# Hi-FT/ERD

Hardware: AMD Instinct MI355X
Metric: images/sec GFL-R50 40+40 incre step @1333x800 (higher is better)
Workload: dtype f32; 1 GPU; gfl_r50_fpn first_40_incre_last_40 ERD (BASELINE configs[1]), 1333x800 padded to 800x1344, fp32, procedural weights; batch_per_gpu=4, global_batch=4, parallelism=dp1

## Files before the change

erd_amd/_lib.py:

```python
from __future__ import annotations

import ctypes as C
import os

_HERE = os.path.dirname(os.path.abspath(__file__))
LIB_PATH = os.environ.get("ERD_HIP_LIB") or os.path.join(_HERE, "lib", "liberd_hip.so")

ERD_MAX_SEG = 5
ERD_MAX_TAPS = 9
ERD_MAX_GROUPS = 8
ERD_SQNORM_PARTS = 1024

c_float_p = C.c_void_p
i64 = C.c_int64
i32 = C.c_int
f32 = C.c_float


class ConvSeg(C.Structure):
    _fields_ = [("inp", C.c_void_p), ("out", C.c_void_p), ("res", C.c_void_p), ("alpha", C.c_void_p),
                ("mask", C.c_void_p), ("N", i32), ("IH", i32), ("IW", i32), ("GH", i32), ("GW", i32), ("OH", i32), ("OW", i32),
                ("in_nstride", i64), ("out_nstride", i64), ("res_nstride", i64),
                ("tap0", i32), ("ntaps", i32), ("oy", i32), ("ox", i32)]


class ConvDesc(C.Structure):
    _fields_ = [("nseg", i32), ("seg", ConvSeg * ERD_MAX_SEG), ("w", C.c_void_p),
                ("Cin", i32), ("Cout", i32), ("wrow", i32), ("ntaps", i32),
                ("dy", i32 * ERD_MAX_TAPS), ("dx", i32 * ERD_MAX_TAPS), ("wk", i32 * ERD_MAX_TAPS),
                ("in_stride", i32), ("out_stride", i32), ("oy", i32), ("ox", i32),
                ("scale", C.c_void_p), ("shift", C.c_void_p), ("relu", i32), ("colsum", C.c_void_p),
                ("sk_ws", C.c_void_p), ("sk_ws_bytes", C.c_size_t), ("w_bf16", C.c_void_p), ("colsum_copies", i32),
                ("in_bf16", i32), ("out_bf16", i32), ("w_x3", C.c_void_p)]


class WgradSeg(C.Structure):
    _fields_ = [("x_off", i64), ("dz_off", i64),
                ("N", i32), ("IH", i32), ("IW", i32), ("GH", i32), ("GW", i32), ("OH", i32), ("OW", i32),
                ("x_nstride", i64), ("dz_nstride", i64)]


class WgradDesc(C.Structure):
    _fields_ = [("x", C.c_void_p), ("dz", C.c_void_p), ("x_elems", i64), ("dz_elems", i64),
                ("nseg", i32), ("seg", WgradSeg * ERD_MAX_SEG),
                ("Cin", i32), ("Cout", i32), ("ntaps", i32),
                ("dy", i32 * ERD_MAX_TAPS), ("dx", i32 * ERD_MAX_TAPS),
                ("in_stride", i32), ("out_stride", i32), ("oy", i32), ("ox", i32),
                ("part", C.c_void_p), ("nsplit", i32), ("bf16_multiplicands", i32),
                ("x_bf16", i32), ("dz_bf16", i32), ("limbs3", i32),
                ("ngroups", i32), ("gx", C.c_void_p * ERD_MAX_GROUPS), ("gdz", C.c_void_p * ERD_MAX_GROUPS)]


class ConvGroupedDesc(C.Structure):
    _fields_ = [("inp", C.c_void_p), ("out", C.c_void_p), ("w", C.c_void_p), ("scale", C.c_void_p), ("shift", C.c_void_p),
                ("res", C.c_void_p), ("mask", C.c_void_p), ("colsum", C.c_void_p), ("colsum_copies", i32),
                ("N", i32), ("IH", i32), ("IW", i32), ("OH", i32), ("OW", i32),
                ("C", i32), ("cg", i32), ("stride", i32), ("relu", i32)]


class WgradReduceGroups(C.Structure):
    _fields_ = [("ngroups", i32), ("w", C.c_void_p * ERD_MAX_GROUPS), ("rowscale", C.c_void_p * ERD_MAX_GROUPS),
                ("dW", C.c_void_p * ERD_MAX_GROUPS), ("rowdot", C.c_void_p * ERD_MAX_GROUPS)]


class BnFoldItem(C.Structure):
    _fields_ = [("gamma", C.c_void_p), ("beta", C.c_void_p), ("mean", C.c_void_p), ("var", C.c_void_p),
                ("scale", C.c_void_p), ("shift", C.c_void_p), ("n", i32), ("eps", f32)]


class WeightPrepItem(C.Structure):
    _fields_ = [("w", C.c_void_p), ("rowscale", C.c_void_p), ("dst", C.c_void_p),
                ("Cout", i32), ("ntaps", i32), ("Cin", i32), ("flip", i32), ("kind", i32), ("block0", i32)]


class ResizeItem(C.Structure):
    _fields_ = [("offset", i64), ("sh", i32), ("sw", i32), ("nh", i32), ("nw", i32), ("flip", i32), ("reserved", i32)]


class Levels(C.Structure):
    _fields_ = [("nseg", i32), ("off", i64 * ERD_MAX_SEG), ("cnt", i64 * ERD_MAX_SEG)]


P = C.c_void_p
_SIGNATURES = {
    "erd_set_cu_reserve": [i32],
    "erd_usable_cus": [],
    "erd_conv_igemm": [C.POINTER(ConvDesc), P],
    "erd_conv_igemm_ws_bytes": [i32],
    "erd_to_bf16": [P, P, i64, P],
    "erd_split3": [P, P, i64, P],
    "erd_conv_thin_enable": [i32],
    "erd_conv_thin_ok": [C.POINTER(ConvDesc)],
    "erd_weight_transpose_x3": [P, P, P, i32, i32, i32, i32, P],
    "erd_wino_weights_elems": [i32, i32],
    "erd_wino_weights": [P, P, i32, i32, i32, P],
    "erd_wino_conv3x3": [P, i32, P, i32, i32, P, P, i32, P, i32, P, P],
    "erd_wino_weights_x3_elems": [i32, i32],
    "erd_wino_weights_x3": [P, P, i32, i32, i32, P],
    "erd_wino_conv3x3_x3": [P, i32, P, i32, i32, P, P, i32, P, i32, P, P],
    "erd_wino_x3_couts_per_item": [P, i32, i32],
    "erd_wino_conv3x3_x3_gn": [P, i32, P, i32, i32, P, P, i32, P, P, C.c_size_t, P],
    "erd_wino_gn_finalize": [P, i32, i32, P, P, f32, P],
    "erd_wino_x3_gn_ws_bytes": [P, i32, i32],
    "erd_conv_wgrad": [C.POINTER(WgradDesc), P],
    "erd_wgrad_row3_slices": [C.POINTER(WgradDesc)],
    "erd_conv_grouped_fwd": [C.POINTER(ConvGroupedDesc), P],
    "erd_conv_grouped_dgrad": [C.POINTER(ConvGroupedDesc), P],
    "erd_conv_grouped_wgrad": [P, P, P, i32, i32, i32, i32, i32, i32, i32, P],
    "erd_conv_grouped_wgrad_splits": [i32, i32, i32, i32, i32, i32],
    "erd_deform_cols": [P, P, P, i32, i32, i32, i32, i32, P],
    "erd_deform_cols_bwd": [P, P, P, P, P, i32, i32, i32, i32, i32, P],
    "erd_wgrad_reduce": [P, i32, i32, i32, P, P, P, i32, P, P],
    "erd_wgrad_reduce_rows": [P, i32, i32, i32, i32, P, i32, P],
    "erd_wgrad_reduce_grouped": [P, i32, i32, i32, C.POINTER(WgradReduceGroups), i32, P],
    "erd_conv_wgrad_wino": [C.POINTER(WgradDesc), P],
    "erd_conv_wgrad_wino_ok": [C.POINTER(WgradDesc)],
    "erd_conv_wgrad_wino_tile": [C.POINTER(WgradDesc)],
    "erd_wgrad_wino_reduce": [P, i32, i32, i32, P, i32, P],
    "erd_weight_transpose": [P, P, P, i32, i32, i32, i32, P],
    "erd_weight_transpose_bf16": [P, P, P, i32, i32, i32, i32, P],
    "erd_stem_conv7x7_bn_relu": [P, P, P, P, P, i32, i32, i32, P],
    "erd_maxpool3x3s2": [P, P, i32, i32, i32, i32, i32, P],
    "erd_bn_fold": [P, P, P, P, f32, P, P, i64, P],
    "erd_bn_fold_batch": [P, i32, i32, P],
    "erd_weight_prep_blocks": [i32, i32, i32, i32],
    "erd_weight_prep_batch": [P, i32, i32, P],
    "erd_relu_bwd_colsum": [P, P, P, i64, i32, i64, i64, P, i32, i32, P],
    "erd_bn_dgamma": [P, P, i32, P, P, f32, P, P, i32, i32, P],
    "erd_gn_relu_fwd": [P, P, P, P, P, P, i32, i64, i32, i32, C.POINTER(Levels), f32, i32, P],
    "erd_gn_relu_apply": [P, P, P, P, P, i32, i64, i32, i32, C.POINTER(Levels), i32, P],
    "erd_gn_relu_bwd": [P, P, P, P, P, P, P, P, P, i32, i64, i32, i32, C.POINTER(Levels), i32, P],
    "erd_upsample2x_add": [P, P, i32, i32, i32, i32, i32, i32, i64, i64, i32, P],
    "erd_upsample2x_add_bwd": [P, P, i32, i32, i32, i32, i32, i32, i64, i64, i32, P],
    "erd_colsum": [P, i64, i32, P, i32, i32, P],
    "erd_pad_channels": [P, P, i64, i32, i32, P],
    "erd_level_scale": [P, P, P, i32, i64, i32, C.POINTER(Levels), P],
    "erd_level_scale_bwd": [P, P, P, P, P, i32, i64, i32, C.POINTER(Levels), P],
    "erd_sgd_momentum": [P, P, P, i64, f32, f32, f32, f32, i32, P],
    "erd_sgd_groups_table": [P, P, P, i32, P, P],
    "erd_sgd_momentum_groups": [P, P, P, i64, i64, P, i32, i32, i64, i64, f32, f32, f32, P, i32, P],
    "erd_adam_groups": [P, P, P, P, i64, i64, P, i32, i32, i64, i64, f32, f32, C.c_double, C.c_double, f32, f32, f32, f32, P, i32, P],
    "erd_grad_sqnorm": [P, i64, P, P],
    "erd_clip_coef": [P, i32, f32, f32, P, P],
    "erd_grad_accumulate": [P, P, i64, i32, P],
    "erd_ers_select": [P, P, i32, i64, i32, i32, P, P, P, P, P, P, P, P],
    "erd_grid_anchors": [P, C.POINTER(i32), C.POINTER(i32), C.POINTER(i32), i32, i32, P],
    "erd_atss_assign": [P, P, C.POINTER(i64), i32, i64, P, P, P, i32, i32, i32, i32, P, P, P, P, P, P],
    "erd_gfl_losses_fwd": [P, P, P, P, P, P, C.POINTER(i64), C.POINTER(i32), i32, i32, i64, i32, i32, P, P, P, P],
    "erd_gfl_losses_bwd": [P, P, P, P, P, P, C.POINTER(i64), C.POINTER(i32), i32, i32, i64, i32, i32, P, P, P, P,
                           P, P],
    "erd_l2_distill": [P, P, P, P, i32, i64, i32, i32, i32, P, P],
    "erd_l2_distill_bwd": [P, P, P, P, P, i32, i64, i32, i32, i32, P, P],
    "erd_distill_nms": [P, P, P, P, P, i32, i64, i32, f32, P, P, P, C.c_size_t, P],
    "erd_kd_kl": [P, P, P, P, i32, i64, i32, i32, f32, P, P],
    "erd_kd_kl_bwd": [P, P, P, P, P, i32, i64, i32, i32, f32, P, P],
    "erd_loss_avg": [P, i32, P, i32, P, P],
    "erd_loss_finalize": [P, P, P, P, P, i32, i32, i32, f32, f32, f32, f32, f32, P, P, P, P],
    "erd_preprocess_image": [P, i32, i32, i32, P, i32, i32, P, P, i32, f32, P],
    "erd_resize_normalize": [P, i32, i32, P, P, P, P, i32, i32, P, i32, i32, P, P, i32, i32, f32, P],
    "erd_resize_normalize_batch": [P, i64, P, i32, P, i32, i32, P, P, i32, f32, P],
    "erd_predict_ws_bytes": [i32, i32, i32],
    "erd_predict_topk": [P, P, P, i32, i64, i32, P, P, P, f32, i32, P, P, P, P, P, C.c_size_t, P],
    "erd_predict_nms": [P, P, P, P, i32, i32, P, f32, f32, i32, P, P, P, P, C.c_size_t, P],
    "erd_tta_merge_ws_bytes": [i32, i32, i32],
    "erd_tta_merge": [P, P, P, i32, i32, i32, P, P, f32, i32, P, P, P, P, C.c_size_t, P],
    "erd_coco_dets_append": [P, P, P, P, i32, i32, P, P, P, P, P],
    "erd_coco_eval_ws_bytes": [i64, i32, i32, i64],
    "erd_coco_eval": [P, P, P, P, i64, P, P, P, P, i32, i32, i64, P, P, P, P, P, P, P, P, C.c_size_t, P],
    "erd_qfl_rows": [P, P, P, i64, i32, P, P],
    "erd_qfl_bwd": [P, P, P, P, i64, i32, P, P],
    "erd_dfl": [P, P, P, i64, i32, P, P, P],
    "erd_kd_kl_rows": [P, P, P, i64, i32, f32, P, P, P],
    "erd_giou": [P, P, P, i64, f32, P, P, P],
    "erd_bbox_overlaps": [P, P, i64, i64, i32, i32, f32, P, P],
    "erd_integral": [P, P, i64, i32, P, P, P],
    "erd_distance2bbox": [P, P, P, i64, f32, f32, P, P, P],
    "erd_bbox2distance": [P, P, i64, f32, f32, P, P],
    "erd_weighted_sum": [P, P, i64, C.c_double, P, P],
    "erd_loss_coef": [P, P, i64, f32, P, P],
    "erd_rows_mul": [P, P, i64, f32, P, P],
    "erd_atss_result": [P, P, i64, P, P, P, P],
}

EXPORTS = ["erd_abi_version", "erd_probe_build", "erd_last_error", "erd_csrc_sha"] + sorted(_SIGNATURES)

_lib = None


class ErdHipError(RuntimeError):
    pass


def load():
    global _lib
    if _lib is not None:
        return _lib
    if not os.path.isfile(LIB_PATH):
        raise ErdHipError(
            f"{LIB_PATH} is missing: build it with `python -c 'import __graft_entry__ as g; g.build()'` "
            "(or `make -C erd_amd/csrc`).  erd_amd has no CPU fallback.")
    lib = C.CDLL(LIB_PATH)
    lib.erd_abi_version.restype = C.c_int
    lib.erd_last_error.restype = C.c_char_p
    lib.erd_csrc_sha.restype = C.c_char_p
    for name, args in _SIGNATURES.items():
        fn = getattr(lib, name)
        fn.argtypes = args
        fn.restype = C.c_size_t if name.endswith(("_ws_bytes", "_elems")) else C.c_int
    if lib.erd_abi_version() != 6:
        raise ErdHipError("liberd_hip.so ABI version mismatch")
    lib.erd_probe_build.restype = C.c_int
    if lib.erd_probe_build() and not os.environ.get("ERD_HIP_LIB"):
        raise ErdHipError(f"{LIB_PATH} is a PROBE build (a kernel was compiled with a timing / accuracy / trace macro of "
                          "csrc/erd_probes.h): rebuild with `make -C erd_amd/csrc`, or select it explicitly with ERD_HIP_LIB")
    _lib = lib
    return lib


def call(name: str, *args) -> None:
    lib = load()
    rc = getattr(lib, name)(*args)
    if rc != 0:
        raise ErdHipError(f"{name} failed (rc={rc}): {lib.erd_last_error().decode(errors='replace')}")
```

erd_amd/csrc/wgrad_wino.hip:

```cpp
#include <stdlib.h>
#include "erd_common.h"

namespace {

typedef float f32x16 __attribute__((ext_vector_type(16)));
typedef __bf16 bf16x8 __attribute__((ext_vector_type(8)));
typedef unsigned int u4v __attribute__((ext_vector_type(4)));
typedef unsigned int u2v __attribute__((ext_vector_type(2)));

constexpr int WT = 512;
constexpr int KT = 16;
constexpr int BC = 128;
constexpr int ROWB = 2 * KT;
constexpr int PLANE = BC * ROWB;
constexpr int LIMB = 2 * PLANE;
constexpr int POS = 3 * LIMB;
constexpr int OPER_BYTES = 4 * POS;
constexpr int TAB_U = 8, NSLOT = 4;
constexpr size_t LDS_BYTES = OPER_BYTES + NSLOT * KT * TAB_U * sizeof(unsigned);
constexpr unsigned INV = 0x80000000u;

__device__ __forceinline__ float2 buf_load8(__amdgpu_buffer_rsrc_t r, unsigned byte_off) {
    const u2v v = __builtin_amdgcn_raw_buffer_load_b64(r, byte_off, 0, 0);
    return make_float2(__uint_as_float(v.x), __uint_as_float(v.y));
}
__device__ __forceinline__ float2 buf_load8(__amdgpu_buffer_rsrc_t r, unsigned byte_off, unsigned uniform_off) {
    const u2v v = __builtin_amdgcn_raw_buffer_load_b64(r, byte_off, uniform_off, 0);
    return make_float2(__uint_as_float(v.x), __uint_as_float(v.y));
}
__device__ __forceinline__ float comp(const float2& v, int c) { return c == 0 ? v.x : v.y; }

struct WinoMap { int xb, zb, IH, IW, OH, OW; };

__device__ __forceinline__ int tiles_w(const erd_wgrad_seg& g) { return (g.GW + 1) >> 1; }
__device__ __forceinline__ int tiles_h(const erd_wgrad_seg& g) { return (g.GH + 1) >> 1; }

struct Sel {
    int xa, xb, za;
    float sx, sz, cz;
    bool z_two;
    __device__ __forceinline__ explicit Sel(int r)
        : xa(r), xb(r < 2 ? 2 : 1), za(r == 3 ? 1 : 0), sx(r == 1 ? 1.f : -1.f), sz(r == 2 ? -1.f : 1.f), cz(r == 1 || r == 2 ? 0.5f : 1.f),
          z_two(r == 1 || r == 2) {}
};

struct TileTable {
    const erd_wgrad_desc& p;
    const Sel& rs;
    const Sel& cs;
    unsigned* tab;
    int lane, ntiles;
    int sl, sn = 0, sa = 0, sb = 0;
    __device__ __forceinline__ TileTable(const erd_wgrad_desc& p_, const Sel& rs_, const Sel& cs_, unsigned* tab_, int lane_, int ntiles_)
        : p(p_), rs(rs_), cs(cs_), tab(tab_), lane(lane_), ntiles(ntiles_), sl(p_.nseg) {}

    __device__ __forceinline__ void tile_entry(const WinoMap& m, int ty, int tx, unsigned (&ent)[5]) const {
        const int ra = 2 * ty - 1 + rs.xa, rb = 2 * ty - 1 + rs.xb, c0 = 2 * tx - 1;
        if ((unsigned)ra < (unsigned)m.IH) ent[0] = (unsigned)(m.xb + (ra * m.IW + c0) * p.Cin) * 4u;
        if ((unsigned)rb < (unsigned)m.IH) ent[1] = (unsigned)(m.xb + (rb * m.IW + c0) * p.Cin) * 4u;
        const int qa = 2 * ty + rs.za, qb = 2 * ty + 1;
        if (qa < m.OH) ent[2] = (unsigned)(m.zb + (qa * m.OW + 2 * tx) * p.Cout) * 4u;
        if (rs.z_two && qb < m.OH) ent[3] = (unsigned)(m.zb + (qb * m.OW + 2 * tx) * p.Cout) * 4u;
        unsigned mask = 0;
#pragma unroll
        for (int b = 0; b < 4; ++b) mask |= (unsigned)(c0 + b) < (unsigned)m.IW ? 1u << b : 0u;
        mask |= (2 * tx < m.OW ? 16u : 0u) | (2 * tx + 1 < m.OW ? 32u : 0u);
        ent[4] = mask;
    }
    __device__ __forceinline__ void tile_entry_pos(const WinoMap& m, int ty, int tx, unsigned (&ent)[8]) const {
        const int ra = 2 * ty - 1 + rs.xa, rb = 2 * ty - 1 + rs.xb, ca = 2 * tx - 1 + cs.xa, cb = 2 * tx - 1 + cs.xb;
        const bool ra_in = (unsigned)ra < (unsigned)m.IH, rb_in = (unsigned)rb < (unsigned)m.IH;
        const bool ca_in = (unsigned)ca < (unsigned)m.IW, cb_in = (unsigned)cb < (unsigned)m.IW;
        if (ra_in && ca_in) ent[0] = (unsigned)(m.xb + (ra * m.IW + ca) * p.Cin) * 4u;
        if (ra_in && cb_in) ent[1] = (unsigned)(m.xb + (ra * m.IW + cb) * p.Cin) * 4u;
        if (rb_in && ca_in) ent[2] = (unsigned)(m.xb + (rb * m.IW + ca) * p.Cin) * 4u;
        if (rb_in && cb_in) ent[3] = (unsigned)(m.xb + (rb * m.IW + cb) * p.Cin) * 4u;
        const int qa = 2 * ty + rs.za, qb = 2 * ty + 1, ka = 2 * tx + cs.za, kb = 2 * tx + 1;
        const bool qb_in = rs.z_two && qb < m.OH, kb_in = cs.z_two && kb < m.OW;
        if (qa < m.OH && ka < m.OW) ent[4] = (unsigned)(m.zb + (qa * m.OW + ka) * p.Cout) * 4u;
        if (qa < m.OH && kb_in) ent[5] = (unsigned)(m.zb + (qa * m.OW + kb) * p.Cout) * 4u;
        if (qb_in && ka < m.OW) ent[6] = (unsigned)(m.zb + (qb * m.OW + ka) * p.Cout) * 4u;
        if (qb_in && kb_in) ent[7] = (unsigned)(m.zb + (qb * m.OW + kb) * p.Cout) * 4u;
    }
    static __device__ __forceinline__ WinoMap map_of(const erd_wgrad_seg& g, int n) {
        return WinoMap{(int)(g.x_off + n * g.x_nstride), (int)(g.dz_off + n * g.dz_nstride), g.IH, g.IW, g.OH, g.OW};
    }
    __device__ __forceinline__ void locate(int u, int& l, int& n, int& a, int& b) const {
        l = 0;
#pragma unroll 1
        for (; l < p.nseg - 1; ++l) {
            const int cnt = p.seg[l].N * tiles_h(p.seg[l]) * tiles_w(p.seg[l]);
            if (u < cnt) break;
            u -= cnt;
        }
        const int TW = tiles_w(p.seg[l]), THW = tiles_h(p.seg[l]) * TW;
        n = u / THW;
        const int rem = u - n * THW;
        a = rem / TW;
        b = rem - a * TW;
    }
    __device__ __forceinline__ void start(int g) {
        if (g * KT < ntiles) locate(g * KT, sl, sn, sa, sb);
    }
    template <bool POS, int SPAN = KT>
    __device__ __forceinline__ void build(int g, int slot) {
        sl = __builtin_amdgcn_readfirstlane(sl);
        sn = __builtin_amdgcn_readfirstlane(sn);
        sa = __builtin_amdgcn_readfirstlane(sa);
        sb = __builtin_amdgcn_readfirstlane(sb);
        if (lane < SPAN) {
            unsigned ent[8] = {INV, INV, INV, INV, POS ? INV : 0u, INV, INV, INV};
            auto entry = [&](const WinoMap& m, int a, int b) {
                if constexpr (POS) tile_entry_pos(m, a, b, ent);
                else tile_entry(m, a, b, reinterpret_cast<unsigned (&)[5]>(ent));
            };
            if (sl < p.nseg) {
                const erd_wgrad_seg& sg = p.seg[sl];
                const int TW = tiles_w(sg);
                int a = sa, b = sb + lane;
                while (b >= TW) { b -= TW; ++a; }
                if (a < tiles_h(sg)) entry(map_of(sg, sn), a, b);
                else if (g * KT + lane < ntiles) {
                    int l, n;
                    locate(g * KT + lane, l, n, a, b);
                    entry(map_of(p.seg[l], n), a, b);
                }
            }
            unsigned* e = tab + (slot * KT + lane) * TAB_U;
            *reinterpret_cast<u4v*>(e) = u4v{ent[0], ent[1], ent[2], ent[3]};
            if constexpr (POS) *reinterpret_cast<u4v*>(e + 4) = u4v{ent[4], ent[5], ent[6], ent[7]};
            else e[4] = ent[4];
        }
        sb += SPAN;
        while (sl < p.nseg && sb >= tiles_w(p.seg[sl])) {
            sb -= tiles_w(p.seg[sl]);
            const bool img = sa + 1 == tiles_h(p.seg[sl]);
            sa = img ? 0 : sa + 1;
            const bool seg = img && sn + 1 == p.seg[sl].N;
            sn = seg ? 0 : sn + (img ? 1 : 0);
            sl += seg ? 1 : 0;
        }
    }
};

__global__ __launch_bounds__(WT) void conv_wgrad_wino_kernel(const erd_wgrad_desc p, const int ntiles, const int nsteps) {
    extern __shared__ __attribute__((aligned(16))) char smem[];
    unsigned* tab = reinterpret_cast<unsigned*>(smem + OPER_BYTES);

    const int tid = threadIdx.x, wave = tid >> 6, lane = tid & 63;
    const int wave_u = __builtin_amdgcn_readfirstlane(wave);

    const int nci = p.Cin / BC, nco = p.Cout / BC, ncomb = 4 * nci * nco;
    const int wg = erd::xcd_contiguous(blockIdx.x, gridDim.x);
    const int split = wg / ncomb, comb = wg - split * ncomb;
    const int r = comb & 3, ct = comb >> 2;
    const int ci0 = (ct % nci) * BC, co0 = (ct / nci) * BC;
    const int per = (nsteps + p.nsplit - 1) / p.nsplit;
    const int g_begin = split * per, g_end = min(nsteps, g_begin + per);

    const Sel rs(r);
    const float sx = rs.sx, sz = rs.sz, cz = rs.cz;
    const bool z_two = rs.z_two;
    TileTable tt{p, rs, rs, tab, lane, ntiles};

    const int cg = (wave & 3) * 16 + (lane & 15), tp = (wave >> 2) * 4 + (lane >> 4);
    const __amdgpu_buffer_rsrc_t rs_x = __builtin_amdgcn_make_buffer_rsrc(const_cast<float*>(p.x), 0, (int)(p.x_elems * 4), 0x00020000);
    const __amdgpu_buffer_rsrc_t rs_z = __builtin_amdgcn_make_buffer_rsrc(const_cast<float*>(p.dz), 0, (int)(p.dz_elems * 4), 0x00020000);
    const unsigned chan_x = (unsigned)(ci0 + 2 * cg) * 4u, chan_z = (unsigned)(co0 + 2 * cg) * 4u;
    const unsigned step_x = (unsigned)p.Cin * 4u, step_z = (unsigned)p.Cout * 4u;
    float2 rx[16], rz[8];
#pragma unroll
    for (int i = 0; i < 8; ++i) rz[i] = make_float2(0.f, 0.f);
    auto load_global = [&](int slot) {
#pragma unroll
        for (int q = 0; q < 2; ++q) {
            const unsigned* e = tab + (slot * KT + 2 * tp + q) * TAB_U;
            const u4v o = *reinterpret_cast<const u4v*>(e);
            const unsigned mask = e[4];
#pragma unroll
            for (int w = 0; w < 2; ++w)
#pragma unroll
                for (int b = 0; b < 4; ++b) {
                    const bool ok = o[w] != INV && ((mask >> b) & 1u);
                    rx[q * 8 + w * 4 + b] = buf_load8(rs_x, ok ? o[w] + (unsigned)b * step_x + chan_x : INV);
                }
#pragma unroll
            for (int w = 0; w < 2; ++w) {
                if (w == 1 && !z_two) continue;
#pragma unroll
                for (int b = 0; b < 2; ++b) {
                    const bool ok = o[2 + w] != INV && ((mask >> (4 + b)) & 1u);
                    rz[q * 4 + w * 2 + b] = buf_load8(rs_z, ok ? o[2 + w] + (unsigned)b * step_z + chan_z : INV);
                }
            }
        }
    };
    char* const st_base = smem + cg * ROWB + ((((tp >> 2) ^ (cg >> 3)) & 1) << 4) + ((tp & 3) << 2);
    auto store_limbs = [&](char* dst, const float (&v)[2][4]) {
#pragma unroll
        for (int j = 0; j < 4; ++j) {
            unsigned hi, mid, lo;
            erd::limbs3_pair(v[0][j], v[1][j], hi, mid, lo);
            *reinterpret_cast<unsigned*>(dst + j * POS) = hi;
            *reinterpret_cast<unsigned*>(dst + j * POS + LIMB) = mid;
            *reinterpret_cast<unsigned*>(dst + j * POS + 2 * LIMB) = lo;
        }
    };
    auto store_lds = [&]() {
#pragma unroll
        for (int c = 0; c < 2; ++c) {
            float v[2][4];
#pragma unroll
            for (int q = 0; q < 2; ++q) {
                float t[4];
#pragma unroll
                for (int b = 0; b < 4; ++b) t[b] = __builtin_fmaf(sx, comp(rx[q * 8 + 4 + b], c), comp(rx[q * 8 + b], c));
                v[q][0] = t[0] - t[2];
                v[q][1] = t[1] + t[2];
                v[q][2] = t[2] - t[1];
                v[q][3] = t[3] - t[1];
            }
            store_limbs(st_base + PLANE + c * (64 * ROWB), v);
#pragma unroll
            for (int q = 0; q < 2; ++q) {
                float t[2];
#pragma unroll
                for (int b = 0; b < 2; ++b) t[b] = cz * __builtin_fmaf(sz, comp(rz[q * 4 + 2 + b], c), comp(rz[q * 4 + b], c));
                v[q][0] = t[0];
                v[q][1] = 0.5f * (t[0] + t[1]);
                v[q][2] = 0.5f * (t[0] - t[1]);
                v[q][3] = t[1];
            }
            store_limbs(st_base + c * (64 * ROWB), v);
        }
    };

    const int pj = wave & 3, half = wave >> 2;
    const int li = lane & 31, h = lane >> 5;
    f32x16 acc[2][4];
#pragma unroll
    for (int i = 0; i < 2; ++i)
#pragma unroll
        for (int j = 0; j < 4; ++j)
#pragma unroll
            for (int e = 0; e < 16; ++e) acc[i][j][e] = 0.f;

    if (g_begin < g_end) {
        if (wave_u == 0) {
            tt.start(g_begin);
            tt.build<false>(g_begin, 0);
            tt.build<false>(g_begin + 1, 1);
        }
        __syncthreads();
        load_global(0);
        store_lds();
        __syncthreads();
        const char* const fr = smem + pj * POS + li * ROWB + (((h ^ (li >> 3)) & 1) << 4);
        for (int g = g_begin; g < g_end; ++g) {
            const int k = g - g_begin;
            const bool more = g + 1 < g_end;
#ifndef ERD_WW_NOLOAD
            if (more) load_global((k + 1) & (NSLOT - 1));
#endif
#ifndef ERD_WW_NOTABLE
            if (wave_u == 0 && g + 2 < g_end) tt.build<false>(g + 2, (k + 2) & (NSLOT - 1));
#endif
#ifndef ERD_WW_NOMFMA
            u4v fa[2][3];
#pragma unroll
            for (int pl = 0; pl < 3; ++pl)
#pragma unroll
                for (int i = 0; i < 2; ++i) fa[i][pl] = *reinterpret_cast<const u4v*>(fr + pl * LIMB + (half * 2 + i) * (32 * ROWB));
#pragma unroll
            for (int jh = 0; jh < 2; ++jh) {
                u4v fb[2][3];
#pragma unroll
                for (int pl = 0; pl < 3; ++pl)
#pragma unroll
                    for (int j = 0; j < 2; ++j) fb[j][pl] = *reinterpret_cast<const u4v*>(fr + pl * LIMB + PLANE + (jh * 2 + j) * (32 * ROWB));
#define ERD_W3(APL, BPL)                                                                                                                     \
    _Pragma("unroll") for (int j = 0; j < 2; ++j) _Pragma("unroll") for (int i = 0; i < 2; ++i) acc[i][jh * 2 + j] =                         \
        __builtin_amdgcn_mfma_f32_32x32x16_bf16(__builtin_bit_cast(bf16x8, fa[i][APL]), __builtin_bit_cast(bf16x8, fb[j][BPL]), acc[i][jh * 2 + j], 0, 0, 0);
                ERD_W3(0, 2) ERD_W3(0, 1) ERD_W3(1, 1) ERD_W3(2, 0) ERD_W3(1, 0) ERD_W3(0, 0)
#undef ERD_W3
            }
#endif
            __syncthreads();
#ifndef ERD_WW_NOSPLIT
            if (more) store_lds();
#endif
            __syncthreads();
        }
    }

    float* __restrict__ part = p.part + ((int64_t)(split * 16 + 4 * r + pj) * p.Cout) * p.Cin;
#pragma unroll
    for (int i = 0; i < 2; ++i)
#pragma unroll
        for (int e = 0; e < 16; ++e) {
            const int co = co0 + 2 * (32 * i + (e & 3) + 8 * (e >> 2) + 4 * h) + half;
            float* row = part + (int64_t)co * p.Cin + ci0 + 2 * li;
            *reinterpret_cast<float2*>(row) = make_float2(acc[i][0][e], acc[i][2][e]);
            *reinterpret_cast<float2*>(row + 64) = make_float2(acc[i][1][e], acc[i][3][e]);
        }
}

constexpr int BP = 256;
constexpr int PPLANE = BP * ROWB;
constexpr int PLIMB = 2 * PPLANE;
constexpr int POPER_BYTES = 3 * PLIMB;
constexpr unsigned PBUF_XOR = 65536;
constexpr int PSPAN = 4 * KT, PNSLOT = 8;
constexpr size_t PTAB_BYTES = PNSLOT * KT * TAB_U * sizeof(unsigned);
constexpr size_t PLDS_BYTES = PBUF_XOR + POPER_BYTES;
static_assert(POPER_BYTES + PTAB_BYTES <= PBUF_XOR, "the table lies between the buffers");

__global__ __launch_bounds__(WT) void wgrad_wino_pos_kernel(const erd_wgrad_desc p, const int ntiles, const int nsteps) {
    extern __shared__ __attribute__((aligned(16))) char smem[];
    unsigned* tab = reinterpret_cast<unsigned*>(smem + POPER_BYTES);

    const int tid = threadIdx.x, wave = tid >> 6, lane = tid & 63;
    const int wave_u = __builtin_amdgcn_readfirstlane(wave);

    const int nci = p.Cin / BP, nco = p.Cout / BP, ncomb = 16 * nci * nco;
    const int wg = erd::xcd_contiguous(blockIdx.x, gridDim.x);
    const int split = wg / ncomb, comb = wg - split * ncomb;
    const int xi = comb & 15, ct = comb >> 4;
    const int ci0 = (ct % nci) * BP, co0 = (ct / nci) * BP;
    const int per = (nsteps + p.nsplit - 1) / p.nsplit;
    const int g_begin = split * per, g_end = min(nsteps, g_begin + per);

    const Sel rs(xi >> 2), cs(xi & 3);
    const float sx = rs.sx, sz = rs.sz, cz = rs.cz;
    const bool z_two = rs.z_two, zc_two = cs.z_two;
    const float sxc = cs.sx, szc = cs.sz;
    TileTable tt{p, rs, cs, tab, lane, ntiles};

    const int cg = wave * 16 + (lane & 15), tq = lane >> 4;
    const __amdgpu_buffer_rsrc_t rs_x = __builtin_amdgcn_make_buffer_rsrc(const_cast<float*>(p.x), 0, (int)(p.x_elems * 4), 0x00020000);
    const __amdgpu_buffer_rsrc_t rs_z = __builtin_amdgcn_make_buffer_rsrc(const_cast<float*>(p.dz), 0, (int)(p.dz_elems * 4), 0x00020000);
    const unsigned chan = (unsigned)cg * 8u, tile_x = (unsigned)ci0 * 4u, tile_z = (unsigned)co0 * 4u;
    float2 rx[16], rz[16];
#pragma unroll
    for (int i = 0; i < 16; ++i) rz[i] = make_float2(0.f, 0.f);
    auto load_global = [&](int slot) {
        u4v ox[4], oz[4];
#pragma unroll
        for (int q = 0; q < 4; ++q) {
            const unsigned* e = tab + (slot * KT + 4 * tq + q) * TAB_U;
            ox[q] = *reinterpret_cast<const u4v*>(e);
            oz[q] = *reinterpret_cast<const u4v*>(e + 4);
        }
#pragma unroll
        for (int q = 0; q < 4; ++q)
#pragma unroll
            for (int i = 0; i < 4; ++i) rx[q * 4 + i] = buf_load8(rs_x, ox[q][i] + chan, tile_x);
#pragma unroll
        for (int q = 0; q < 4; ++q) rz[q * 4] = buf_load8(rs_z, oz[q][0] + chan, tile_z);
        if (zc_two) {
#pragma unroll
            for (int q = 0; q < 4; ++q) rz[q * 4 + 1] = buf_load8(rs_z, oz[q][1] + chan, tile_z);
        }
        if (z_two) {
#pragma unroll
            for (int q = 0; q < 4; ++q) rz[q * 4 + 2] = buf_load8(rs_z, oz[q][2] + chan, tile_z);
            if (zc_two) {
#pragma unroll
                for (int q = 0; q < 4; ++q) rz[q * 4 + 3] = buf_load8(rs_z, oz[q][3] + chan, tile_z);
            }
        }
    };
    unsigned st_off = cg * ROWB + ((((tq >> 1) ^ (cg >> 3)) & 1) << 4) + ((tq & 1) << 3);
    auto store_limbs = [&](char* dst, const float (&v)[4]) {
        unsigned hi[2], mid[2], lo[2];
        erd::limbs3_pair(v[0], v[1], hi[0], mid[0], lo[0]);
        erd::limbs3_pair(v[2], v[3], hi[1], mid[1], lo[1]);
        *reinterpret_cast<u2v*>(dst) = u2v{hi[0], hi[1]};
        *reinterpret_cast<u2v*>(dst + PLIMB) = u2v{mid[0], mid[1]};
        *reinterpret_cast<u2v*>(dst + 2 * PLIMB) = u2v{lo[0], lo[1]};
    };
    auto store_lds = [&]() {
        char* const st = smem + st_off;
#pragma unroll
        for (int c = 0; c < 2; ++c) {
            float v[4];
#pragma unroll
            for (int q = 0; q < 4; ++q) {
                const float ta = __builtin_fmaf(sx, comp(rx[q * 4 + 2], c), comp(rx[q * 4], c));
                const float tb = __builtin_fmaf(sx, comp(rx[q * 4 + 3], c), comp(rx[q * 4 + 1], c));
                v[q] = __builtin_fmaf(sxc, tb, ta);
            }
            store_limbs(st + PPLANE + c * (128 * ROWB), v);
#pragma unroll
            for (int q = 0; q < 4; ++q) {
                const float ta = cz * __builtin_fmaf(sz, comp(rz[q * 4 + 2], c), comp(rz[q * 4], c));
                const float tb = cz * __builtin_fmaf(sz, comp(rz[q * 4 + 3], c), comp(rz[q * 4 + 1], c));
                v[q] = zc_two ? 0.5f * __builtin_fmaf(szc, tb, ta) : ta;
            }
            store_limbs(st + c * (128 * ROWB), v);
        }
    };

    const int zq = wave >> 1, hx = wave & 1;
    const int li = lane & 31, h = lane >> 5;
    f32x16 acc[2][4];
#pragma unroll
    for (int i = 0; i < 2; ++i)
#pragma unroll
        for (int j = 0; j < 4; ++j)
#pragma unroll
            for (int e = 0; e < 16; ++e) acc[i][j][e] = 0.f;

    if (g_begin < g_end) {
        if (wave_u == 0) {
            tt.start(g_begin);
            tt.build<true, PSPAN>(g_begin, 0);
            tt.build<true, PSPAN>(g_begin + 4, 4);
        }
        __syncthreads();
        load_global(0);
        store_lds();
        __syncthreads();
        st_off ^= PBUF_XOR;
        unsigned fr_off = li * ROWB + (((h ^ (li >> 3)) & 1) << 4);
        for (int g = g_begin; g < g_end; ++g) {
            const int k = g - g_begin;
            const bool more = g + 1 < g_end;
            const char* const fr = smem + fr_off;
#ifndef ERD_WW_NOLOAD
            if (more) load_global((k + 1) & (PNSLOT - 1));
#endif
#ifndef ERD_WW_NOTABLE
            if (wave_u == 0 && (k & 3) == 3 && g + 5 < g_end) tt.build<true, PSPAN>(g + 5, (k + 5) & (PNSLOT - 1));
#endif
#ifndef ERD_WW_NOMFMA
            u4v fa[2][3];
#pragma unroll
            for (int pl = 0; pl < 3; ++pl)
#pragma unroll
                for (int i = 0; i < 2; ++i) fa[i][pl] = *reinterpret_cast<const u4v*>(fr + pl * PLIMB + (zq * 2 + i) * (32 * ROWB));
#pragma unroll
            for (int j = 0; j < 4; ++j) {
                u4v fb[3];
#pragma unroll
                for (int pl = 0; pl < 3; ++pl)
                    fb[pl] = *reinterpret_cast<const u4v*>(fr + pl * PLIMB + PPLANE + (2 * hx + (j & 1) + 4 * (j >> 1)) * (32 * ROWB));
#define ERD_W3(APL, BPL)                                                                                                                     \
    _Pragma("unroll") for (int i = 0; i < 2; ++i) acc[i][j] =                                                                                \
        __builtin_amdgcn_mfma_f32_32x32x16_bf16(__builtin_bit_cast(bf16x8, fa[i][APL]), __builtin_bit_cast(bf16x8, fb[BPL]), acc[i][j], 0, 0, 0);
                ERD_W3(0, 2) ERD_W3(0, 1) ERD_W3(1, 1) ERD_W3(2, 0) ERD_W3(1, 0) ERD_W3(0, 0)
#undef ERD_W3
            }
#endif
#ifndef ERD_WW_NOSPLIT
            if (more) store_lds();
#endif
            __syncthreads();
            fr_off ^= PBUF_XOR;
            st_off ^= PBUF_XOR;
        }
    }

    float* __restrict__ part = p.part + ((int64_t)(split * 16 + xi) * p.Cout) * p.Cin;
#pragma unroll
    for (int i = 0; i < 2; ++i)
#pragma unroll
        for (int e = 0; e < 16; ++e) {
            const int co = co0 + 2 * (32 * (2 * (zq & 1) + i) + (e & 3) + 8 * (e >> 2) + 4 * h) + (zq >> 1);
            float* row = part + (int64_t)co * p.Cin + ci0 + 2 * (64 * hx + li);
            *reinterpret_cast<float2*>(row) = make_float2(acc[i][0][e], acc[i][2][e]);
            *reinterpret_cast<float2*>(row + 64) = make_float2(acc[i][1][e], acc[i][3][e]);
        }
}

__global__ __launch_bounds__(256) void wgrad_wino_reduce_kernel(const float* __restrict__ part, int nsplit, int Cout, int Cin,
                                                                 float* __restrict__ dW, int accumulate) {
    __shared__ float4 du[16][16];
    const int co = blockIdx.x, xi = threadIdx.x >> 4, c4 = threadIdx.x & 15;
    const int ci = blockIdx.y * 64 + c4 * 4;
    const int64_t slab = (int64_t)16 * Cout * Cin;
    float4 s = make_float4(0.f, 0.f, 0.f, 0.f);
    if (ci < Cin) {
        const float* src = part + ((int64_t)xi * Cout + co) * Cin + ci;
        for (int k = 0; k < nsplit; ++k) {
            const float4 v = *reinterpret_cast<const float4*>(src + k * slab);
            s.x += v.x; s.y += v.y; s.z += v.z; s.w += v.w;
        }
    }
    du[xi][c4] = s;
    __syncthreads();
    if (threadIdx.x >= 9 * 16 || ci >= Cin) return;
    const int a = xi / 3, b = xi - 3 * a;
    auto col = [&](int i) {
        const float4 u1 = du[4 * i + 1][c4], u2 = du[4 * i + 2][c4];
        if (b == 1) return make_float4(u1.x - u2.x, u1.y - u2.y, u1.z - u2.z, u1.w - u2.w);
        const float4 u0 = du[4 * i + (b == 0 ? 0 : 3)][c4];
        return make_float4((u1.x + u2.x) + u0.x, (u1.y + u2.y) + u0.y, (u1.z + u2.z) + u0.z, (u1.w + u2.w) + u0.w);
    };
    const float4 e1 = col(1), e2 = col(2);
    float4 o;
    if (a == 1) o = make_float4(e1.x - e2.x, e1.y - e2.y, e1.z - e2.z, e1.w - e2.w);
    else {
        const float4 e0 = col(a == 0 ? 0 : 3);
        o = make_float4((e1.x + e2.x) + e0.x, (e1.y + e2.y) + e0.y, (e1.z + e2.z) + e0.z, (e1.w + e2.w) + e0.w);
    }
    float* dst = dW + ((int64_t)co * 9 + xi) * Cin + ci;
    if (accumulate) {
        const float4 old = *reinterpret_cast<const float4*>(dst);
        o.x += old.x; o.y += old.y; o.z += old.z; o.w += old.w;
    }
    *reinterpret_cast<float4*>(dst) = o;
}

int64_t wino_tiles(const erd_wgrad_desc* d) {
    int64_t n = 0;
    for (int l = 0; l < d->nseg; ++l) n += (int64_t)d->seg[l].N * ((d->seg[l].GH + 1) / 2) * ((d->seg[l].GW + 1) / 2);
    return n;
}

int wino_tile(const erd_wgrad_desc* d) {
    const bool can = d->Cin % BP == 0 && d->Cout % BP == 0;
    const char* const e = getenv("ERD_WGRAD_WINO_TILE");
    const int force = e ? atoi(e) : 0;
    if (force == BC || !can) return BC;
    return BP;
}

}

extern "C" int erd_conv_wgrad_wino_tile(const erd_wgrad_desc* d) { return erd_conv_wgrad_wino_ok(d) ? wino_tile(d) : 0; }

extern "C" int erd_conv_wgrad_wino_ok(const erd_wgrad_desc* d) {
    if (!d || d->bf16_multiplicands || d->x_bf16 || d->dz_bf16 || d->ngroups != 1) return 0;
    if (d->nseg < 1 || d->nseg > ERD_MAX_SEG || d->Cin < BC || d->Cout < BC || d->Cin % BC || d->Cout % BC) return 0;
    if (d->x_elems <= 0 || d->dz_elems <= 0 || d->x_elems >= (1ll << 29) || d->dz_elems >= (1ll << 29)) return 0;
    for (int l = 0; l < d->nseg; ++l)
        if (d->seg[l].N < 1 || d->seg[l].GH < 1 || d->seg[l].GW < 1) return 0;
    return erd_wgrad_row3_slices(d) > 0 && wino_tiles(d) < (1ll << 30);
}

extern "C" int erd_conv_wgrad_wino(const erd_wgrad_desc* d, erd_stream_t stream) {
    ERD_REQUIRE(d != nullptr && d->part && d->x && d->dz, "wgrad_wino: null pointer");
    ERD_REQUIRE(!d->bf16_multiplicands && !d->x_bf16 && !d->dz_bf16, "wgrad_wino: fp32 maps and the three-limb form only");
    ERD_REQUIRE(d->ngroups == 1, "wgrad_wino: ngroups=%d", d->ngroups);
    ERD_REQUIRE(d->Cin >= BC && d->Cout >= BC && d->Cin % BC == 0 && d->Cout % BC == 0, "wgrad_wino: Cin=%d Cout=%d must be multiples of %d", d->Cin,
                d->Cout, BC);
    ERD_REQUIRE(d->in_stride == 1 && d->out_stride == 1, "wgrad_wino: stride 1 only");
    ERD_REQUIRE(erd_conv_wgrad_wino_ok(d), "wgrad_wino: not a 3x3 / stride 1 / pad 1 layer over 1 .. %d non-empty maps below 2 GiB", ERD_MAX_SEG);
    const int64_t grid = (int64_t)4 * (d->Cin / BC) * (d->Cout / BC) * d->nsplit;
    ERD_REQUIRE(d->nsplit >= 1 && grid < (1 << 20), "wgrad_wino: nsplit=%d", d->nsplit);
    const int ntiles = (int)wino_tiles(d), nsteps = (ntiles + KT - 1) / KT;
    static bool attr_done = false;
    if (!attr_done) {
        (void)hipFuncSetAttribute(reinterpret_cast<const void*>(conv_wgrad_wino_kernel), hipFuncAttributeMaxDynamicSharedMemorySize, (int)LDS_BYTES);
        (void)hipFuncSetAttribute(reinterpret_cast<const void*>(wgrad_wino_pos_kernel), hipFuncAttributeMaxDynamicSharedMemorySize, (int)PLDS_BYTES);
        attr_done = true;
    }
    if (wino_tile(d) == BP) hipLaunchKernelGGL(wgrad_wino_pos_kernel, dim3((unsigned)grid), dim3(WT), PLDS_BYTES, (hipStream_t)stream, *d, ntiles, nsteps);
    else hipLaunchKernelGGL(conv_wgrad_wino_kernel, dim3((unsigned)grid), dim3(WT), LDS_BYTES, (hipStream_t)stream, *d, ntiles, nsteps);
    return erd::check_launch("conv_wgrad_wino");
}

extern "C" int erd_wgrad_wino_reduce(const float* part, int nsplit, int Cout, int Cin, float* dW, int accumulate, erd_stream_t stream) {
    ERD_REQUIRE(part && dW && nsplit >= 1 && Cout >= 1 && Cin >= 4 && Cin % 4 == 0, "wgrad_wino_reduce: bad args");
    hipLaunchKernelGGL(wgrad_wino_reduce_kernel, dim3(Cout, (Cin + 63) / 64), dim3(256), 0, (hipStream_t)stream, part, nsplit, Cout, Cin, dW,
                       accumulate & 1);
    return erd::check_launch("wgrad_wino_reduce");
}
```

erd_amd/functional.py:

```python
from __future__ import annotations

from typing import List, Optional, Sequence, Tuple

import torch
from torch.autograd import Function

from . import kernels as K

Tensor = torch.Tensor


def ohwi(w: Tensor) -> Tensor:
    v = w.detach().permute(0, 2, 3, 1)
    if not v.is_contiguous():
        return v.contiguous()
    v._erd_owner = w
    return v


def _to_oihw(dw_ohwi: Tensor) -> Tensor:
    return dw_ohwi.permute(0, 3, 1, 2)


_AUX = {}
import contextlib as _contextlib
import os as _os
WGRAD_ON_AUX_STREAM = _os.environ.get('ERD_WGRAD_AUX', '0') != '0'
TOWERS_ON_TWO_STREAMS = _os.environ.get('ERD_TOWER_AUX', '1') != '0'


_TOWER = {}

CAPTURE_ORIGIN = None


def _may_fork(cur) -> bool:
    return CAPTURE_ORIGIN is None or cur.cuda_stream == CAPTURE_ORIGIN


WGRAD_TRAIL = _os.environ.get('ERD_WGRAD_TRAIL', '1') != '0'
WGRAD_GROUPED = _os.environ.get('ERD_WGRAD_GROUPED', '1') != '0'
WGRAD_WINO = _os.environ.get('ERD_WGRAD_WINO', '1') != '0'
WGRAD_GROUP_CAP = 8
RES_LAYER_NODE = _os.environ.get('ERD_RES_LAYER', '1') != '0'
HEAD_TRAIL = _os.environ.get('ERD_HEAD_TRAIL', '0') != '0'
_TRAIL = {}
_TRAIL_ACTIVE = set()


def trail_stream(device) -> "torch.cuda.Stream":
    key = str(torch.device(device))
    if key not in _TRAIL:
        _TRAIL[key] = torch.cuda.Stream(device=device)
    return _TRAIL[key]


def trail_join(device=None) -> None:
    for key in list(_TRAIL_ACTIVE):
        if device is None or key == str(torch.device(device)):
            torch.cuda.current_stream(torch.device(key)).wait_stream(_TRAIL[key])
            _TRAIL_ACTIVE.discard(key)


class _Trail:

    def __init__(self, device, *tensors):
        self.cur = torch.cuda.current_stream(device)
        self.aux = trail_stream(device)
        self.tensors = [t for t in tensors if t is not None]
        self.key = str(torch.device(device))
        self.inline = not _may_fork(self.cur)

    def __enter__(self):
        if self.inline:
            return self
        self.aux.wait_stream(self.cur)
        for t in self.tensors:
            t.record_stream(self.aux)
        _TRAIL_ACTIVE.add(self.key)
        self.ctx = torch.cuda.stream(self.aux)
        self.ctx.__enter__()
        return self

    def __exit__(self, *a):
        if not self.inline:
            self.ctx.__exit__(*a)
        return False


def aux_stream(device) -> "torch.cuda.Stream":
    cur = torch.cuda.current_stream(device)
    if not TOWERS_ON_TWO_STREAMS or not _may_fork(cur):
        return cur
    key = (str(device), cur.cuda_stream)
    if key not in _TOWER:
        _TOWER[key] = torch.cuda.Stream(device=device)
    return _TOWER[key]


class _Fork:
    def __init__(self, device):
        self.cur = torch.cuda.current_stream(device)
        key = (str(device), self.cur.cuda_stream)
        if key not in _AUX:
            _AUX[key] = torch.cuda.Stream(device=device)
        self.aux = _AUX[key] if WGRAD_ON_AUX_STREAM and _may_fork(self.cur) else None

    def __enter__(self):
        if self.aux is not None:
            self.aux.wait_stream(self.cur)
            self.ctx = torch.cuda.stream(self.aux)
            self.ctx.__enter__()
        return self

    def __exit__(self, *a):
        if self.aux is not None:
            self.ctx.__exit__(*a)
        return False

    def join(self):
        if self.aux is not None:
            self.cur.wait_stream(self.aux)


def _sink(p: Optional[Tensor]) -> Optional[Tensor]:
    if p is not None and getattr(p, "_erd_sink", False) and p.grad is not None:
        return p.grad
    return None


def _sunk(p: Tensor) -> None:
    n = getattr(p, "_erd_sink_notify", None)
    if n is not None:
        n(p)


def _emit_wgrad(w: Tensor, part: Tensor, S: int, wk: Tensor, scale: Optional[Tensor], rowdot: Optional[Tensor]):
    sink = _sink(w)
    if sink is not None:
        K.wgrad_reduce(part, S, wk, scale, ohwi(sink), True, rowdot, rowdot_zeroed=True)
        _sunk(w)
        return None
    dWk = torch.empty_like(wk)
    K.wgrad_reduce(part, S, wk, scale, dWk, False, rowdot, rowdot_zeroed=True)
    return _to_oihw(dWk)


def _emit_wgrad_wino(w: Tensor, part: Tensor, S: int, wk: Tensor):
    sink = _sink(w)
    if sink is not None:
        K.wgrad_wino_reduce(part, S, ohwi(sink), True)
        _sunk(w)
        return None
    dWk = torch.empty_like(wk)
    K.wgrad_wino_reduce(part, S, dWk, False)
    return _to_oihw(dWk)


class _WgradGroups:

    def __init__(self, device, eps: float):
        self.dev, self.eps, self.keys = device, eps, {}
        self.launches = []

    @staticmethod
    def takes(xin: Tensor, dz: Tensor, cardinality: int = 1) -> bool:
        if cardinality > 1:
            return False
        return WGRAD_GROUPED and CAPTURE_ORIGIN is None and K.COMPUTE == "f32x3" and K.WGRAD_X3 and K.WGRAD_X3_GENERIC and xin.dtype == torch.float32 \
            and dz.dtype == torch.float32 and _os.environ.get("ERD_WGRAD_ROW3", "1") != "0"

    def add(self, single, xin, dz, k, s, pad, scale, dbeta, prm, need3) -> None:
        key = (k, s, pad, xin.shape, xin.stride(), dz.shape, dz.stride())
        q = self.keys.setdefault(key, [])
        q.append((single, xin, dz, k, s, pad, scale, dbeta, prm, need3))
        if len(q) == WGRAD_GROUP_CAP:
            self._launch(self.keys.pop(key))

    def flush(self) -> None:
        for key in list(self.keys):
            self._launch(self.keys.pop(key))

    def _launch(self, q) -> None:
        self.launches.append(len(q))
        if len(q) == 1:
            q[0][0]()
            return
        _, _, _, k, s, pad = q[0][:6]
        with (_Trail(self.dev, *[t for m in q for t in (m[1], m[2], m[6], m[7])]) if WGRAD_TRAIL else _contextlib.nullcontext()):
            part, S = K.conv_wgrad_partials_grouped([[m[1]] for m in q], [[m[2]] for m in q], k, s, pad)
            wks = [ohwi(m[8][0]) for m in q]
            rowdots = [K.zeros_f32(m[6].numel(), m[6].device) if m[9][1] else None for m in q]
            K.wgrad_reduce_grouped(part, S, wks, [m[6] for m in q], [ohwi(_sink(m[8][0])) for m in q], True, rowdots, rowdot_zeroed=True)
            for m, rowdot in zip(q, rowdots):
                (w, g, b, mean, var), (_, need_g, need_b), dbeta = m[8], m[9], m[7]
                _sunk(w)
                if need_g:
                    rep = dbeta.dim() == 2
                    bs_fold = (_sink(b) if need_b else None) if rep else None
                    fold = None if not rep else (bs_fold if bs_fold is not None else torch.empty_like(dbeta[0]))
                    K.bn_dgamma(rowdot, dbeta, mean, var, self.eps, out=_sink(g), dbeta_out=fold)
                    _sunk(g)
                    if rep:
                        dbeta = fold
                elif dbeta.dim() == 2:
                    dbeta = dbeta.sum(0)
                if need_b:
                    bs = _sink(b)
                    if dbeta.data_ptr() != bs.data_ptr():
                        bs.add_(dbeta)
                    _sunk(b)


def _bn_fold_cached(gamma, beta, mean, var, eps):
    if gamma.requires_grad or beta.requires_grad:
        pre = getattr(gamma, "_erd_prefold", None)
        if pre is not None and pre[0] == (gamma.data_ptr(), beta.data_ptr(), mean.data_ptr(), var.data_ptr(), gamma._version,
                                         beta._version, mean._version, var._version, eps) and pre[1][0]:
            return pre[2], pre[3]
        return K.bn_fold(gamma.detach(), beta.detach(), mean, var, eps)
    ver = (gamma.data_ptr(), beta.data_ptr(), mean.data_ptr(), var.data_ptr(),
           gamma._version, beta._version, mean._version, var._version, eps)
    hit = getattr(gamma, "_erd_fold", None)
    if hit is None or hit[0] != ver:
        hit = (ver, K.bn_fold(gamma.detach(), beta.detach(), mean, var, eps))
        gamma._erd_fold = hit
    return hit[1]


class BnPrefold:

    def __init__(self, model):
        from ._lib import BnFoldItem
        bns = [m for m in model.modules() if hasattr(m, "running_var") and hasattr(m, "weight") and m.weight is not None
               and (m.weight.requires_grad or m.bias.requires_grad)]
        self.bns = bns
        self.valid = [False]
        if not bns:
            return
        dev = bns[0].weight.device
        total = sum(m.weight.numel() for m in bns)
        self.buf = torch.empty(2 * total, dtype=torch.float32, device=dev)
        items = (BnFoldItem * len(bns))()
        off = 0
        self.views = []
        for it, m in zip(items, bns):
            n = m.weight.numel()
            sc, sh = self.buf[off:off + n], self.buf[total + off:total + off + n]
            it.gamma, it.beta, it.mean, it.var = m.weight.data_ptr(), m.bias.data_ptr(), m.running_mean.data_ptr(), m.running_var.data_ptr()
            it.scale, it.shift, it.n, it.eps = sc.data_ptr(), sh.data_ptr(), n, float(m.eps)
            sc._erd_stable = True
            self.views.append((sc, sh))
            off += n
        import ctypes as C
        raw = bytes(memoryview(items))
        self.table = torch.frombuffer(bytearray(raw), dtype=torch.uint8).to(dev)
        self.max_n = max(m.weight.numel() for m in bns)
        self._ptrs = None

    def run(self) -> None:
        if not self.bns:
            return
        self._run(self.bns, self.views, self.table, self.max_n, None)

    def set_groups(self, group_of) -> None:
        from ._lib import BnFoldItem
        import ctypes as C
        size = C.sizeof(BnFoldItem)
        self.groups, self.gtables, self._gptrs = {}, {}, {}
        if not self.bns:
            return
        for j, m in enumerate(self.bns):
            g = group_of(m.weight)
            self.groups.setdefault(group_of(m.bias) if g is None else g, []).append(j)
        host = self.table.cpu()
        for g, js in self.groups.items():
            sub = torch.cat([host[j * size:(j + 1) * size] for j in js]).to(self.table.device)
            self.gtables[g] = (sub, [self.bns[j] for j in js], [self.views[j] for j in js], max(self.bns[j].weight.numel() for j in js))

    def run_group(self, g: int) -> None:
        ent = self.gtables.get(g)
        if ent is None:
            return
        table, bns, views, max_n = ent
        self._run(bns, views, table, max_n, g)

    def _run(self, bns, views, table, max_n, g) -> None:
        ptrs = tuple((m.weight.data_ptr(), m.bias.data_ptr(), m.running_mean.data_ptr(), m.running_var.data_ptr()) for m in bns)
        seen = self._ptrs if g is None else self._gptrs.get(g)
        if seen is not None and ptrs != seen:
            self.valid[0] = False
            return
        if g is None:
            self._ptrs = ptrs
        else:
            self._gptrs[g] = ptrs
        K.call("erd_bn_fold_batch", K._p(table), len(bns), max_n, K._stream())
        for m, (sc, sh) in zip(bns, views):
            g_, b = m.weight, m.bias
            g_._erd_prefold = ((g_.data_ptr(), b.data_ptr(), m.running_mean.data_ptr(), m.running_var.data_ptr(), g_._version, b._version,
                                m.running_mean._version, m.running_var._version, m.eps), self.valid, sc, sh)
        self.valid[0] = True


def _wgrad_plain(w: Tensor, xs, dzs, k: int, stride: int, pad: int, keep=(), trail: bool = True):
    wk = ohwi(w)
    wino = WGRAD_WINO and (k, stride, pad) == (3, 1, 1) and K.conv_wgrad_wino_ok(xs, dzs)

    def run():
        if wino:
            part, S = K.conv_wgrad_wino(xs, dzs)
            return _emit_wgrad_wino(w, part, S, wk)
        part, S = K.conv_wgrad_partials(xs, dzs, k, stride, pad)
        return _emit_wgrad(w, part, S, wk, None, None)

    if trail and WGRAD_TRAIL and _sink(w) is not None:
        with _Trail(xs[0].device, *(keep or (list(xs) + list(dzs)))):
            return run()
    return run()


class ConvBNAct(Function):

    @staticmethod
    def forward(ctx, x, w, gamma, beta, mean, var, res, k: int, stride: int, pad: int, relu: bool, eps: float):
        K.RECORDED = any(ctx.needs_input_grad)
        wk = ohwi(w)
        scale, shift = _bn_fold_cached(gamma, beta, mean, var, eps)
        N, H, W_, _ = x.shape
        OH, OW = K.conv_out_size(H, k, stride, pad), K.conv_out_size(W_, k, stride, pad)
        out = torch.empty((N, OH, OW, wk.shape[0]), dtype=x.dtype, device=x.device)
        K.conv_forward([x], wk, [out], k, stride, pad, scale=scale, shift=shift,
                       res=None if res is None else [res], relu=relu)
        ctx.cfg = (k, stride, pad, relu, eps, res is not None)
        ctx.save_for_backward(x, w, mean, var, scale, out)
        return out

    @staticmethod
    def backward(ctx, dy):
        x, w, mean, var, scale, out = ctx.saved_tensors
        k, stride, pad, relu, eps, has_res = ctx.cfg
        need_x, need_w, need_g, need_b = ctx.needs_input_grad[0:4]
        dy = dy.contiguous()
        dz, dbeta = K.relu_bwd_colsum(out if relu else None, dy, relu, want_colsum=need_g or need_b)
        wk = ohwi(w)
        card = x.shape[3] // w.shape[1]
        dW = dgamma = None
        fork = _Fork(x.device)
        if need_w or need_g:
            rowdot = K.zeros_f32(scale.numel(), scale.device) if need_g else None
            dgamma = torch.empty_like(scale) if need_g else None
            with fork:
                part, S = K.conv_wgrad_partials([x], [dz], k, stride, pad, cardinality=card)
                dW = _emit_wgrad(w, part, S, wk, scale, rowdot)
                if need_g:
                    K.bn_dgamma(rowdot, dbeta, mean, var, eps, out=dgamma)
        dx = None
        if need_x and card > 1:
            dx = torch.empty_like(x)
            K.conv_dgrad([dz], wk, [dx], k, stride, pad, cardinality=card, rowscale=scale)
        elif need_x:
            wt = K.weight_transpose(wk, scale)
            dx = torch.zeros_like(x) if k < stride else torch.empty_like(x)
            K.conv_dgrad([dz], wt, [dx], k, stride, pad)
        fork.join()
        dres = dz if (has_res and ctx.needs_input_grad[6]) else None
        return dx, dW, dgamma, (dbeta if need_b else None), None, None, dres, None, None, None, None, None


class DeformConvBNAct(Function):

    @staticmethod
    def forward(ctx, x, w, w_off, b_off, gamma, beta, mean, var, stride: int, relu: bool, eps: float):
        K.RECORDED = any(ctx.needs_input_grad)
        K._deform_mode_check("DeformConvBNAct", x)
        wk = ohwi(w)
        scale, shift = _bn_fold_cached(gamma, beta, mean, var, eps)
        x = x.contiguous()
        N, H, W_, _ = x.shape
        OH, OW = K.conv_out_size(H, 3, stride, 1), K.conv_out_size(W_, 3, stride, 1)
        offset = torch.empty((N, OH, OW, 18), dtype=torch.float32, device=x.device)
        K.conv_forward([x], ohwi(w_off), [offset], 3, stride, 1, shift=b_off.detach())
        out = torch.empty((N, OH, OW, wk.shape[0]), dtype=x.dtype, device=x.device)
        K.deform_conv3x3_forward(x, offset, wk, out, stride, scale=scale, shift=shift, relu=relu)
        ctx.cfg = (stride, relu, eps)
        ctx.bias_param = b_off
        ctx.save_for_backward(x, w, w_off, mean, var, scale, out, offset)
        return out

    @staticmethod
    def backward(ctx, dy):
        x, w, w_off, mean, var, scale, out, offset = ctx.saved_tensors
        stride, relu, eps = ctx.cfg
        need_x, need_w, need_wo, need_bo, need_g, need_b = ctx.needs_input_grad[0:6]
        dz, dbeta = K.relu_bwd_colsum(out if relu else None, dy.contiguous(), relu, want_colsum=need_g or need_b)
        wk = ohwi(w)
        dW = dgamma = dWo = dbo = dx = None
        if need_w or need_g:
            rowdot = K.zeros_f32(scale.numel(), scale.device) if need_g else None
            part, S = K.deform_conv3x3_wgrad_partials(x, offset, dz, stride)
            dW = _emit_wgrad(w, part, S, wk, scale, rowdot)
            if need_g:
                dgamma = K.bn_dgamma(rowdot, dbeta, mean, var, eps)
        if need_x or need_wo or need_bo:
            dx = torch.zeros_like(x)
            doffset = K.deform_conv3x3_dgrad(dz, wk, scale, x, offset, stride, dx)
            wok = ohwi(w_off)
            Cp = 32
            dop = K.pad_channels(doffset, Cp)
            if need_wo:
                part, S = K.conv_wgrad_partials([x], [dop], 3, stride, 1)
                sink = _sink(w_off)
                if sink is not None:
                    K.wgrad_reduce_rows(part, S, Cp, ohwi(sink), True)
                    _sunk(w_off)
                else:
                    dWk = torch.empty_like(wok)
                    K.wgrad_reduce_rows(part, S, Cp, dWk, False)
                    dWo = _to_oihw(dWk)
            if need_bo:
                dbo = _bias_grad(ctx.bias_param, doffset)
            if need_x:
                wp = K.pad_channels(wok.reshape(1, -1), Cp * wok[0].numel()).view(Cp, *wok.shape[1:])
                K.conv_dgrad([dop], K.weight_transpose(wp), [dx], 3, stride, 1, accumulate=True)
            else:
                dx = None
        return dx, dW, dWo, dbo, dgamma, (dbeta if need_b else None), None, None, None, None, None


class BottleneckFn(Function):

    @staticmethod
    def forward(ctx, x, stride: int, eps: float, *params):
        K.RECORDED = any(ctx.needs_input_grad)
        has_down = len(params) == 20
        P = [params[5 * i:5 * i + 5] for i in range(4 if has_down else 3)]
        dev = x.device

        def cba(inp, prm, k, s, pad, res, relu):
            w, g, b, m, v = prm
            wk = ohwi(w)
            scale, shift = _bn_fold_cached(g, b, m, v, eps)
            N, H, W_, _ = inp.shape
            out = torch.empty((N, K.conv_out_size(H, k, s, pad), K.conv_out_size(W_, k, s, pad), wk.shape[0]),
                              dtype=inp.dtype, device=dev)
            K.conv_forward([inp], wk, [out], k, s, pad, scale=scale, shift=shift,
                           res=None if res is None else [res], relu=relu)
            return out, scale

        o1, s1 = cba(x, P[0], 1, 1, 0, None, True)
        o2, s2 = cba(o1, P[1], 3, stride, 1, None, True)
        sd = None
        idn = x
        if has_down:
            idn, sd = cba(x, P[3], 1, stride, 0, None, False)
        y, s3 = cba(o2, P[2], 1, 1, 0, idn, True)
        ctx.cfg = (stride, eps, has_down)
        ctx.save_for_backward(x, o1, o2, y, s1, s2, s3, *( [sd] if has_down else []), *params)
        return y

    @staticmethod
    def backward(ctx, dy):
        stride, eps, has_down = ctx.cfg
        saved = ctx.saved_tensors
        x, o1, o2, y, s1, s2, s3 = saved[:7]
        off = 7
        sd = None
        if has_down:
            sd = saved[7]
            off = 8
        params = saved[off:]
        P = [params[5 * i:5 * i + 5] for i in range(4 if has_down else 3)]
        need = ctx.needs_input_grad
        b3 = P[2][2]
        s_ = _sink(b3) if need[3 + 5 * 2 + 2] else None
        dz3, db3 = K.relu_bwd_colsum(y, dy.contiguous(), True, colsum_into=s_ if s_ is not None else K.zeros_f32(y.shape[3], x.device))
        dx, grads = _bottleneck_backward(x, o1, o2, s1, s2, s3, sd, P, list(need[3:]), need[0], stride, eps, dz3, db3)
        return (dx, None, None, *grads)


def _bottleneck_backward(x, o1, o2, s1, s2, s3, sd, P, need_p, need_x, stride, eps, dz3, db3, out_mask=None, groups=None):
    has_down = sd is not None
    dev = x.device
    grads = [None] * (5 * len(P))

    card2 = o1.shape[3] // P[1][0].shape[1]

    def wgrad(idx, xin, dz, k, s, pad, scale, dbeta, collect=True, card=1):
        w, g, b, m, v = P[idx]
        base = 5 * idx
        if not (need_p[base] or need_p[base + 1] or need_p[base + 2]):
            return
        wk = ohwi(w)
        trail = None
        sunk = all((not need_p[base + q]) or _sink(t) is not None for q, t in enumerate((w, g, b)))
        if collect and groups is not None and sunk and need_p[base] and groups.takes(xin, dz, card):
            groups.add(lambda: wgrad(idx, xin, dz, k, s, pad, scale, dbeta, collect=False), xin, dz, k, s, pad, scale, dbeta, (w, g, b, m, v),
                       tuple(need_p[base:base + 3]))
            return
        if WGRAD_TRAIL and sunk:
            trail = _Trail(dev, xin, dz, scale, dbeta)
            trail.__enter__()
        try:
            _wgrad_body(idx, xin, dz, k, s, pad, scale, dbeta, w, g, b, m, v, base, wk, card)
        finally:
            if trail is not None:
                trail.__exit__(None, None, None)

    def _wgrad_body(idx, xin, dz, k, s, pad, scale, dbeta, w, g, b, m, v, base, wk, card=1):
        part, S = K.conv_wgrad_partials([xin], [dz], k, s, pad, cardinality=card)
        rowdot = K.zeros_f32(scale.numel(), scale.device) if need_p[base + 1] else None
        grads[5 * idx] = _emit_wgrad(w, part, S, wk, scale, rowdot)
        if need_p[base + 1]:
            rep = dbeta.dim() == 2
            bs_fold = (_sink(b) if need_p[base + 2] else None) if rep else None
            fold = None if not rep else (bs_fold if bs_fold is not None else torch.empty_like(dbeta[0]))
            gs = _sink(g)
            if gs is not None:
                K.bn_dgamma(rowdot, dbeta, m, v, eps, out=gs, dbeta_out=fold)
                _sunk(g)
            else:
                grads[5 * idx + 1] = K.bn_dgamma(rowdot, dbeta, m, v, eps, dbeta_out=fold)
            if rep:
                dbeta = fold
        elif dbeta.dim() == 2:
            dbeta = dbeta.sum(0)
        if need_p[base + 2]:
            bs = _sink(b)
            if bs is None:
                grads[5 * idx + 2] = dbeta
            else:
                if dbeta.data_ptr() != bs.data_ptr():
                    bs.add_(dbeta)
                _sunk(b)

    wgrad(2, o2, dz3, 1, 1, 0, s3, db3)
    dz2 = torch.empty_like(o2)
    rep_slot = lambda n: K.zeros_f32(K.colsum_copies(n) * n, dev).view(K.colsum_copies(n), n)
    db2 = rep_slot(o2.shape[3])
    K.conv_dgrad([dz3], K.weight_transpose(ohwi(P[2][0]), s3), [dz2], 1, 1, 0, relu_mask=[o2], colsum=db2)
    wgrad(1, o1, dz2, 3, stride, 1, s2, db2, card=card2)
    dz1 = torch.empty_like(o1)
    db1 = rep_slot(o1.shape[3])
    if card2 > 1:
        K.conv_dgrad([dz2], ohwi(P[1][0]), [dz1], 3, stride, 1, relu_mask=[o1], colsum=db1, cardinality=card2, rowscale=s2)
    else:
        K.conv_dgrad([dz2], K.weight_transpose(ohwi(P[1][0]), s2), [dz1], 3, stride, 1, relu_mask=[o1], colsum=db1)
    wgrad(0, x, dz1, 1, 1, 0, s1, db1)
    dx = None
    if need_x:
        dx = torch.empty_like(x)
        wt1 = K.weight_transpose(ohwi(P[0][0]), s1)
        if has_down:
            assert out_mask is None, "the fused ReLU mask needs an identity shortcut (one launch writes every pixel of dx)"
            K.conv_dgrad([dz1], wt1, [dx], 1, 1, 0)
            K.conv_dgrad([dz3], K.weight_transpose(ohwi(P[3][0]), sd), [dx], 1, stride, 0, accumulate=True)
        elif out_mask is not None:
            db_prev = rep_slot(x.shape[3])
            K.conv_dgrad([dz1], wt1, [dx], 1, 1, 0, res=[dz3], relu_mask=[out_mask], colsum=db_prev)
            dx = (dx, db_prev)
        else:
            K.conv_dgrad([dz1], wt1, [dx], 1, 1, 0, res=[dz3])
    if has_down:
        wgrad(3, x, dz3, 1, stride, 0, sd, db3)
    return dx, grads


class ResLayerFn(Function):

    @staticmethod
    def forward(ctx, x, strides, eps: float, counts, *params):
        K.RECORDED = any(ctx.needs_input_grad)
        dev = x.device
        blocks, off = [], 0
        for n in counts:
            blocks.append(params[off:off + n])
            off += n
        saved, meta = [], []

        def cba(inp, prm, k, s, pad, res, relu):
            w, g, b, m, v = prm
            wk = ohwi(w)
            scale, shift = _bn_fold_cached(g, b, m, v, eps)
            N, H, W_, _ = inp.shape
            out = torch.empty((N, K.conv_out_size(H, k, s, pad), K.conv_out_size(W_, k, s, pad), wk.shape[0]),
                              dtype=inp.dtype, device=dev)
            K.conv_forward([inp], wk, [out], k, s, pad, scale=scale, shift=shift,
                           res=None if res is None else [res], relu=relu)
            return out, scale

        h = x
        for bp, stride in zip(blocks, strides):
            has_down = len(bp) == 20
            P = [bp[5 * i:5 * i + 5] for i in range(4 if has_down else 3)]
            o1, s1 = cba(h, P[0], 1, 1, 0, None, True)
            o2, s2 = cba(o1, P[1], 3, stride, 1, None, True)
            sd, idn = None, h
            if has_down:
                idn, sd = cba(h, P[3], 1, stride, 0, None, False)
            y, s3 = cba(o2, P[2], 1, 1, 0, idn, True)
            meta.append((stride, has_down, len(saved)))
            saved += [h, o1, o2, y, s1, s2, s3] + ([sd] if has_down else [])
            h = y
        ctx.meta, ctx.eps, ctx.counts, ctx.nsaved = meta, eps, counts, len(saved)
        ctx.save_for_backward(*saved, *params)
        return h

    @staticmethod
    def backward(ctx, dy):
        saved = ctx.saved_tensors
        acts, params = saved[:ctx.nsaved], saved[ctx.nsaved:]
        need = ctx.needs_input_grad
        blocks, need_b, off = [], [], 0
        for n in ctx.counts:
            blocks.append(params[off:off + n])
            need_b.append(list(need[4 + off:4 + off + n]))
            off += n
        grads_all = [None] * len(params)
        nb = len(blocks)
        dz3 = db3 = None
        dx = None
        groups = _WgradGroups(dy.device, ctx.eps) if WGRAD_GROUPED else None
        for i in range(nb - 1, -1, -1):
            stride, has_down, a0 = ctx.meta[i]
            x, o1, o2, y, s1, s2, s3 = acts[a0:a0 + 7]
            sd = acts[a0 + 7] if has_down else None
            bp = blocks[i]
            P = [bp[5 * j:5 * j + 5] for j in range(4 if has_down else 3)]
            if i == nb - 1:
                b3 = P[2][2]
                s_ = _sink(b3) if need_b[i][5 * 2 + 2] else None
                dz3, db3 = K.relu_bwd_colsum(y, dy.contiguous(), True,
                                             colsum_into=s_ if s_ is not None else K.zeros_f32(y.shape[3], x.device))
            fuse = i > 0 and not has_down
            need_x = need[0] if i == 0 else True
            out, g = _bottleneck_backward(x, o1, o2, s1, s2, s3, sd, P, need_b[i], need_x, stride, ctx.eps, dz3, db3,
                                          out_mask=x if fuse else None, groups=groups)
            base = sum(ctx.counts[:i])
            grads_all[base:base + len(g)] = g
            if i == 0:
                dx = out
            elif fuse:
                dz3, db3 = out
            else:
                prev_y = acts[ctx.meta[i - 1][2] + 3]
                pb3 = blocks[i - 1][5 * 2 + 2]
                s_ = _sink(pb3) if need_b[i - 1][5 * 2 + 2] else None
                dz3, db3 = K.relu_bwd_colsum(prev_y, out, True,
                                             colsum_into=s_ if s_ is not None else K.zeros_f32(prev_y.shape[3], x.device))
        if groups is not None:
            groups.flush()
            ResLayerFn.last_group_launches = groups.launches
        return (dx, None, None, None, *grads_all)


def _bias_grad(b: Tensor, dy: Tensor, rows: Optional[Tensor] = None):
    sink = _sink(b)
    if sink is not None:
        K.colsum(dy if rows is None else rows, out=sink)
        _sunk(b)
        return None
    return K.colsum(dy if rows is None else rows)


class ConvBias(Function):

    @staticmethod
    def forward(ctx, x, w, b, k: int, stride: int, pad: int):
        K.RECORDED = any(ctx.needs_input_grad)
        wk = ohwi(w)
        N, H, W_, _ = x.shape
        OH, OW = K.conv_out_size(H, k, stride, pad), K.conv_out_size(W_, k, stride, pad)
        out = torch.empty((N, OH, OW, wk.shape[0]), dtype=x.dtype, device=x.device)
        K.conv_forward([x], wk, [out], k, stride, pad, shift=b.detach())
        ctx.cfg = (k, stride, pad)
        ctx.bias_param = b
        ctx.save_for_backward(x, w)
        return out

    @staticmethod
    def backward(ctx, dy):
        x, w = ctx.saved_tensors
        k, stride, pad = ctx.cfg
        dy = dy.contiguous()
        wk = ohwi(w)
        dW = db = dx = None
        if ctx.needs_input_grad[1]:
            dW = _wgrad_plain(w, [x], [dy], k, stride, pad)
        if ctx.needs_input_grad[2]:
            db = _bias_grad(ctx.bias_param, dy)
        if ctx.needs_input_grad[0]:
            dx = torch.zeros_like(x) if k < stride else torch.empty_like(x)
            K.conv_dgrad([dy], K.weight_transpose(wk), [dx], k, stride, pad)
        return dx, dW, db, None, None, None


class UpsampleAdd(Function):

    @staticmethod
    def forward(ctx, fine, coarse):
        ctx.mark_dirty(fine)
        K.upsample_add_(fine, coarse)
        ctx.cshape = coarse.shape
        return fine

    @staticmethod
    def backward(ctx, dout):
        dout = dout.contiguous()
        dcoarse = None
        if ctx.needs_input_grad[1]:
            dcoarse = torch.zeros(ctx.cshape, dtype=dout.dtype, device=dout.device)
            K.upsample_add_bwd_(dout, dcoarse)
        return dout, dcoarse


class FPNOutputs(Function):

    @staticmethod
    def forward(ctx, l3, l4, l5, w0, w1, w2, w3, w4, b0, b1, b2, b3, b4):
        K.RECORDED = any(ctx.needs_input_grad)
        lats = [l3, l4, l5]
        ws = [w0, w1, w2, w3, w4]
        bs = [b0, b1, b2, b3, b4]
        N = l3.shape[0]
        sizes = [(l.shape[1], l.shape[2]) for l in lats]
        h, w_ = sizes[-1]
        for _ in range(2):
            h, w_ = K.conv_out_size(h, 3, 2, 1), K.conv_out_size(w_, 3, 2, 1)
            sizes.append((h, w_))
        A = sum(a * b for a, b in sizes)
        Cc = w0.shape[0]
        cat = torch.empty((N, A, Cc), dtype=l3.dtype, device=l3.device)
        views = K.level_views(cat, sizes)
        for i in range(3):
            K.conv_forward([lats[i]], ohwi(ws[i]), [views[i]], 3, 1, 1, shift=bs[i].detach())
        K.conv_forward([views[2]], ohwi(ws[3]), [views[3]], 3, 2, 1, shift=bs[3].detach())
        K.conv_forward([views[3]], ohwi(ws[4]), [views[4]], 3, 2, 1, shift=bs[4].detach())
        ctx.sizes = sizes
        ctx.bias_params = bs
        ctx.save_for_backward(l3, l4, l5, cat, *ws)
        return cat

    @staticmethod
    def backward(ctx, dcat):
        l3, l4, l5, cat, *ws = ctx.saved_tensors
        sizes = ctx.sizes
        lats = [l3, l4, l5]
        dcat = dcat.contiguous()
        dv = list(K.level_views(dcat, sizes))
        dv[3] = dv[3].clone()
        dv[2] = dv[2].clone()
        pv = K.level_views(cat, sizes)
        grads_w: List[Optional[Tensor]] = [None] * 5
        grads_b: List[Optional[Tensor]] = [None] * 5

        def wgrad(i, xin, dz, stride):
            wk = ohwi(ws[i])
            if ctx.needs_input_grad[3 + i]:
                grads_w[i] = _wgrad_plain(ws[i], [xin], [dz], 3, stride, 1, keep=(xin, dcat, dz))
            if ctx.needs_input_grad[8 + i]:
                sink = _sink(ctx.bias_params[i])
                if sink is not None:
                    K.relu_bwd_colsum(None, dz, False, colsum_into=sink)
                    _sunk(ctx.bias_params[i])
                else:
                    grads_b[i] = K.relu_bwd_colsum(None, dz, False)[1]
            return wk

        wk = wgrad(4, pv[3], dv[4], 2)
        K.conv_dgrad([dv[4]], K.weight_transpose(wk), [dv[3]], 3, 2, 1, accumulate=True)
        wk = wgrad(3, pv[2], dv[3], 2)
        K.conv_dgrad([dv[3]], K.weight_transpose(wk), [dv[2]], 3, 2, 1, accumulate=True)
        dl: List[Optional[Tensor]] = [None, None, None]
        for i in range(3):
            wk = wgrad(i, lats[i], dv[i], 1)
            if ctx.needs_input_grad[i]:
                dl[i] = torch.empty_like(lats[i])
                K.conv_dgrad([dv[i]], K.weight_transpose(wk), [dl[i]], 3, 1, 1)
        return (dl[0], dl[1], dl[2], *grads_w, *grads_b)


class HeadConvGN(Function):

    @staticmethod
    def forward(ctx, x_cat, w, gamma, beta, sizes, eps: float):
        K.RECORDED = any(ctx.needs_input_grad)
        c, y, mr = K.conv3x3_gn_relu_forward(x_cat, ohwi(w), gamma.detach(), beta.detach(), sizes, 32, eps)
        ctx.sizes = sizes
        ctx.save_for_backward(x_cat, w, gamma, beta, c, mr)
        return y

    @staticmethod
    def backward(ctx, dy):
        x_cat, w, gamma, beta, c, mr = ctx.saved_tensors
        sizes = ctx.sizes
        gs, bs_ = _sink(gamma), _sink(beta)
        direct = gs is not None and bs_ is not None
        dc, dgamma, dbeta = K.gn_relu_backward(c, dy.contiguous(), gamma.detach(), beta.detach(), mr, sizes, 32,
                                               dgamma=gs if direct else None, dbeta=bs_ if direct else None)
        if direct:
            _sunk(gamma)
            _sunk(beta)
            dgamma = dbeta = None
        wk = ohwi(w)
        dW = dx = None
        xv, dv = K.level_views(x_cat, sizes), K.level_views(dc, sizes)
        if ctx.needs_input_grad[1]:
            dW = _wgrad_plain(w, xv, dv, 3, 1, 1, keep=(x_cat, dc), trail=HEAD_TRAIL)
        if ctx.needs_input_grad[0]:
            dx = torch.empty_like(x_cat)
            K.conv_dgrad(dv, K.weight_transpose(wk), K.level_views(dx, sizes), 3, 1, 1)
        return dx, dW, dgamma, dbeta, None, None


class HeadConvBias(Function):
# ... 115 lines not shown
```

erd_amd/kernels.py:

```python
from __future__ import annotations

import ctypes as C
import os as _os
from typing import Dict, List, Optional, Sequence, Tuple

import torch

from . import _lib
from ._lib import ConvDesc, Levels, WgradDesc, call

Tensor = torch.Tensor


_raw_stream = getattr(torch._C, "_cuda_getCurrentRawStream", None)


def _cur_stream() -> int:
    if _raw_stream is not None:
        return _raw_stream(torch.cuda.current_device())
    return torch.cuda.current_stream().cuda_stream


def _stream() -> C.c_void_p:
    return C.c_void_p(_cur_stream())
# ... 684 lines not shown
    def invalidate(self) -> None:
        self.stamp += 1
        self._stale()

    def _drop_stale(self, items) -> None:
        for key, r in items:
            if r.src.data_ptr() != r.src_ptr or (r.rowscale is not None and r.rowscale.data_ptr() != r.rs_ptr) or \
                    r.owner._version != r.version:
                self.recipes.pop(key, None)
                if key[0] == "T":
                    self.recipes.pop(("UT", key[1]), None)
                    self.recipes.pop(("UT3", key[1]), None)
                    self.recipes.pop(("XT", key[1]), None)
                self._tables = None
                self._gtables = {}
                self._stale()

    def _build_tables(self, recipes) -> list:
        from ._lib import WeightPrepItem
        lib = _lib.load()
        tables = []
        for level in (0, 1):
            rs = [r for r in recipes if r.level == level]
            if not rs:
                continue
            items = (WeightPrepItem * len(rs))()
            blk = 0
            for it, r in zip(items, rs):
                it.w, it.rowscale, it.dst = r.src_ptr, r.rs_ptr, r.out.data_ptr()
                it.Cout, it.ntaps, it.Cin, it.flip, it.kind, it.block0 = r.Cout, r.ntaps, r.Cin, r.flip, r.kind, blk
                blk += int(lib.erd_weight_prep_blocks(r.kind, r.Cout, r.ntaps, r.Cin))
            table = torch.frombuffer(bytearray(bytes(memoryview(items))), dtype=torch.uint8).to(self.device)
            tables.append((table, len(rs), blk, rs))
        return tables

    def run_group(self, g: int) -> None:
        if self.group_of is None:
            raise RuntimeError("ParamPrep.run_group: no group_of")
        if self.stamp == 0:
            self.stamp = 1
        mine = [(k, r) for k, r in self.recipes.items() if self.group_of(r.owner) == g]
        self._drop_stale(mine)
        tables = self._gtables.get(g)
        if tables is None:
            tables = self._gtables[g] = self._build_tables([r for r in self.recipes.values() if self.group_of(r.owner) == g])
        for table, n, blocks, rs in tables:
            call("erd_weight_prep_batch", _p(table), n, blocks, _stream())
            for r in rs:
                r.stamp = self.stamp

    def run(self) -> None:
        self.stamp += 1
        if not self.recipes:
            return
        self._drop_stale(list(self.recipes.items()))
        if self._tables is None:
            self._tables = self._build_tables(list(self.recipes.values()))
        for table, n, blocks, rs in self._tables:
            call("erd_weight_prep_batch", _p(table), n, blocks, _stream())
            for r in rs:
                r.stamp = self.stamp


def _prep_owner(w: Tensor):
    o = getattr(w, "_erd_owner", None)
    return o if o is not None and getattr(o, "_erd_sink", False) else None


def _prep_of(owner) -> Optional[ParamPrep]:
    return None if owner is None else getattr(owner, "_erd_prep", None)


def weight_transpose(w: Tensor, rowscale: Optional[Tensor] = None) -> Tensor:
    Cout, k, _, Cin = w.shape
    bf = COMPUTE == "bf16"
    owner = _prep_owner(w)
    PREP = _prep_of(owner)
    if PREP is None:
        owner = None
    if owner is not None:
        r = PREP.lookup(("T", id(owner), bf))
        if r is not None and r.matches(owner, w, rowscale):
            return r.out
    if bf:
        wt = torch.empty((Cin, k, k, Cout), dtype=torch.bfloat16, device=w.device)
        call("erd_weight_transpose_bf16", _p(w), _p(rowscale), _p(wt), Cout, k * k, Cin, 0, _stream())
    else:
        wt = torch.empty((Cin, k, k, Cout), dtype=torch.float32, device=w.device)
        call("erd_weight_transpose", _p(w), _p(rowscale), _p(wt), Cout, k * k, Cin, 0, _stream())
    if owner is not None and (rowscale is None or getattr(rowscale, "_erd_stable", False)) and not torch.cuda.is_current_stream_capturing():
        PREP.register(("T", id(owner), bf), 1 if bf else 0, w, rowscale, torch.empty_like(wt), Cout, k * k, Cin, 0, owner, 0)
    return wt


def conv_dgrad(dzs: Sequence[Tensor], wt: Tensor, dxs: Sequence[Tensor], k: int, stride: int, pad: int,
               accumulate: bool = False, res: Optional[Sequence[Tensor]] = None,
               relu_mask: Optional[Sequence[Tensor]] = None, colsum: Optional[Tensor] = None, cardinality: int = 1,
               rowscale: Optional[Tensor] = None) -> None:
    _require_gpu(wt, *dzs, *dxs)
    if cardinality > 1:
        if len(dzs) != 1 or k != 3 or pad != 1:
            raise ValueError("grouped convolution: one map, 3x3, pad 1 (ResNeXt conv2)")
        _conv_grouped_dgrad(dzs[0], wt, dxs[0], stride, rowscale, accumulate, None if res is None else res[0],
                            None if relu_mask is None else relu_mask[0], colsum)
        return
    assert rowscale is None, "conv_dgrad: a row scale goes into weight_transpose (cardinality 1)"
    Cin, Cout = wt.shape[0], wt.shape[3]
    if wt.dtype == torch.float32 and WINO_DGRAD and wino_ok(Cout, k, stride, pad):
        wino_conv3x3(dzs, wino_weights(wt, flip=True), dxs, Cin, res=(dxs if accumulate else res), mask=relu_mask,
                     colsum=colsum, kname="conv_wino_dgrad")
        return
    wtb = None
    wtx = None
    if COMPUTE == "bf16":
        wtb = wt if wt.dtype == torch.bfloat16 else to_bf16(wt)
    elif wt.dtype != torch.float32:
        raise ValueError("conv_dgrad: bf16 weights in f32 compute mode")
    elif COMPUTE == "f32x3" and Cout % 4 == 0:
        wtx = _weights_x3(wt, grad_form=True)
    if stride == 2 and k == 3 and len(dzs) == 1 and MERGE_PARITY:
        _dgrad_s2_merged(dzs[0], wt, wtb, dxs[0], pad, Cin, Cout, accumulate, res, relu_mask, colsum, wtx=wtx)
        return
    cache = _desc_cache()
    key = ("dgrad", k, stride, pad, accumulate, wt.shape, _geom(dzs), _geom(dxs), None if res is None else _geom(res),
           None if relu_mask is None else _geom(relu_mask), None if colsum is None else colsum.numel(), COMPUTE)
    ent = cache.get(key)
    if ent is None:
        ent = cache[key] = _dgrad_descs(dzs, wt, dxs, k, stride, pad, accumulate, res, relu_mask, colsum, Cin, Cout)
    for d, flop, nbytes, tag in ent:
        for i in range(len(dzs)):
            sg = d.seg[i]
            sg.inp, sg.out = dzs[i].data_ptr(), dxs[i].data_ptr()
            if accumulate:
                sg.res = dxs[i].data_ptr()
            elif res is not None:
                sg.res = res[i].data_ptr()
            if relu_mask is not None:
                sg.mask = relu_mask[i].data_ptr()
        d.w = wt.data_ptr() if wtb is None else 0
        d.colsum = 0 if colsum is None else colsum.data_ptr()
        if wtb is not None:
            d.w_bf16 = wtb.data_ptr()
        d.w_x3 = 0 if wtx is None else wtx.data_ptr()
        _attach_sk_ws(d, wt.device)
        _timed_call(_igemm_class(d, "dgrad"), flop, "erd_conv_igemm", C.byref(d), _stream(), nbytes=nbytes if _TIMING is not None else 0.0,
                    tag=tag if TIMING_DETAIL else "")


def _dgrad_descs(dzs, wt, dxs, k, stride, pad, accumulate, res, relu_mask, colsum, Cin, Cout):
    out = []
    classes = [(0, 0)] if stride == 1 else [(py, px) for py in range(stride) for px in range(stride)]
    for (py, px) in classes:
        taps = []
        for kh in range(k):
            if (py + pad - kh) % stride:
                continue
            for kw in range(k):
                if (px + pad - kw) % stride:
                    continue
                taps.append(((py + pad - kh) // stride, (px + pad - kw) // stride, (kh * k + kw) * Cout))
        if not taps:
            continue
        d = ConvDesc()
        d.nseg = len(dzs)
        skip = False
        for i, (dz, dx) in enumerate(zip(dzs, dxs)):
            assert dz.shape[3] == Cout and dx.shape[3] == Cin
            GH = (dx.shape[1] - py + stride - 1) // stride
            GW = (dx.shape[2] - px + stride - 1) // stride
            if GH <= 0 or GW <= 0:
                skip = True
            r = dx if accumulate else (None if res is None else res[i])
            _fill_seg(d.seg[i], dz, dx, max(GH, 0), max(GW, 0), r, None, None if relu_mask is None else relu_mask[i])
        if skip and len(dzs) == 1:
            continue
        d.Cin, d.Cout, d.wrow = Cout, Cin, k * k * Cout
        d.ntaps = len(taps)
        for t, (dy, dx_, wk) in enumerate(taps):
            d.dy[t], d.dx[t], d.wk[t] = dy, dx_, wk
        d.in_stride, d.out_stride, d.oy, d.ox = 1, stride, py, px
        d.scale = 0
        d.shift = 0
        d.relu = 0
        d.colsum_copies = 0 if colsum is None else colsum.numel() // Cin
        d.in_bf16, d.out_bf16 = _stored_bf16(dzs), _stored_bf16(dxs, res, relu_mask)
        flop = 2.0 * sum(d.seg[i].N * d.seg[i].GH * d.seg[i].GW for i in range(d.nseg)) * Cin * len(taps) * Cout
        nbytes = 4.0 * (sum(t.numel() for t in dzs) + sum(t.numel() for t in dxs) / (stride * stride) + wt.numel() /
                        (stride * stride))
        out.append((d, flop, nbytes, _shape_tag(d, k, stride) + f" class{py}{px}"))
    return out


MERGE_PARITY = _os.environ.get("ERD_MERGE_PARITY", "1") != "0"


def _dgrad_s2_merged(dz: Tensor, wt: Tensor, wtb, dx: Tensor, pad: int, Cin: int, Cout: int, accumulate: bool, res,
                     relu_mask, colsum, wtx=None) -> None:
    k, stride = 3, 2
    d = ConvDesc()
    nseg, tap0, flop = 0, 0, 0.0
    for (py, px) in ((1, 1), (0, 1), (1, 0), (0, 0)):
        taps = [((py + pad - kh) // stride, (px + pad - kw) // stride, (kh * k + kw) * Cout)
                for kh in range(k) if (py + pad - kh) % stride == 0
                for kw in range(k) if (px + pad - kw) % stride == 0]
        GH = (dx.shape[1] - py + stride - 1) // stride
        GW = (dx.shape[2] - px + stride - 1) // stride
        if not taps or GH <= 0 or GW <= 0:
            continue
        sg = d.seg[nseg]
        r = dx if accumulate else (None if res is None else res[0])
        _fill_seg(sg, dz, dx, GH, GW, r, None, None if relu_mask is None else relu_mask[0])
        sg.tap0, sg.ntaps, sg.oy, sg.ox = tap0, len(taps), py, px
        for t, (dy, dx_, wk) in enumerate(taps):
            d.dy[tap0 + t], d.dx[tap0 + t], d.wk[tap0 + t] = dy, dx_, wk
        tap0 += len(taps)
        flop += 2.0 * sg.N * GH * GW * Cin * len(taps) * Cout
        nseg += 1
    if nseg == 0:
        return
    d.nseg = nseg
    d.ntaps = max(d.seg[i].ntaps for i in range(nseg))
    d.w = wt.data_ptr() if wtb is None else 0
    d.Cin, d.Cout, d.wrow = Cout, Cin, k * k * Cout
    d.in_stride, d.out_stride, d.oy, d.ox = 1, stride, 0, 0
    d.scale = d.shift = 0
    d.relu = 0
    d.colsum = 0 if colsum is None else colsum.data_ptr()
    d.colsum_copies = 0 if colsum is None else colsum.numel() // Cin
    if wtb is not None:
        d.w_bf16 = wtb.data_ptr()
    d.w_x3 = 0 if wtx is None else wtx.data_ptr()
    d.in_bf16, d.out_bf16 = _stored_bf16([dz]), _stored_bf16([dx], res, relu_mask)
    d.sk_ws, d.sk_ws_bytes = 0, 0
    nbytes = 4.0 * (dz.numel() + dx.numel() + wt.numel()) if _TIMING is not None else 0.0
    _timed_call("conv_igemm_dgrad", flop, "erd_conv_igemm", C.byref(d), _stream(), nbytes=nbytes,
                tag=(_shape_tag(d, k, stride) + " merged") if TIMING_DETAIL else "")


def _shape_tag(d, k: int, stride: int) -> str:
    px = sum(d.seg[i].N * d.seg[i].GH * d.seg[i].GW for i in range(d.nseg))
    return f"px{px} {d.Cin}->{d.Cout} k{k}s{stride}"


WGRAD_X3_GENERIC = _os.environ.get("ERD_WGRAD_X3_GENERIC", "1") != "0"
WGRAD_X3 = _os.environ.get("ERD_WGRAD_X3", "1") != "0"


CU_RESERVE = 0


def set_cu_reserve(n: int) -> int:
    global CU_RESERVE
    prev = int(_lib.load().erd_set_cu_reserve(int(n)))
    CU_RESERVE = int(n)
    return prev


def _one_round(target: int) -> int:
    if CU_RESERVE == 0:
        return target
    usable = int(_lib.load().erd_usable_cus())
    return max(1, target * usable // (usable + CU_RESERVE))


def _pick_nsplit(npix: int, Cout: int, Cin: int, ntaps: int) -> int:
    tiles = ((Cout + 127) // 128) * ((Cin + 127) // 128) * ntaps
    kt = (npix + 31) // 32
    dflt = "512" if COMPUTE == "bf16" else "1024"
    target = _one_round(int(dflt) if _os.environ.get("ERD_WGRAD_VARIANT", "1") == "0" else int(_os.environ.get("ERD_WGRAD_TARGET", dflt)))
    want = max(1, target // tiles)
    return int(max(1, min(want, kt // 8 if kt >= 8 else 1, 512)))


def _extent(t: Tensor):
    last = sum((sz - 1) * st for sz, st in zip(t.shape, t.stride()))
    return t.data_ptr(), last + 1


def conv_wgrad_partials(xs: Sequence[Tensor], dzs: Sequence[Tensor], k: int, stride: int, pad: int, cardinality: int = 1):
    _require_gpu(*xs, *dzs)
    if cardinality > 1:
        if len(xs) != 1 or k != 3 or pad != 1:
            raise ValueError("grouped convolution: one map, 3x3, pad 1 (ResNeXt conv2)")
        return _conv_grouped_wgrad_partials(xs[0], dzs[0], stride, cardinality)
    xb = min(x.data_ptr() for x in xs)
    zb = min(z.data_ptr() for z in dzs)
    xoff = tuple((x.data_ptr() - xb) // x.element_size() for x in xs)
    zoff = tuple((z.data_ptr() - zb) // z.element_size() for z in dzs)
    cache = _desc_cache()
    key = ("wgrad", k, stride, pad, _geom(xs), _geom(dzs), xoff, zoff, COMPUTE, _os.environ.get("ERD_WGRAD_ROW3", "1"), WGRAD_X3, WGRAD_X3_GENERIC,
           CU_RESERVE)
    ent = cache.get(key)
    if ent is None:
        ent = cache[key] = _wgrad_desc(xs, dzs, k, stride, pad, xoff, zoff)
    d, S, flop, nbytes, tag, Cout, Cin, row3 = ent
    d.x, d.dz = xb, zb
    part = ws_float("wgrad_part", S * Cout * k * k * Cin, xs[0].device)
    d.part = part.data_ptr()
    _timed_call("conv_wgrad_row3" if row3 else "conv_wgrad", flop, "erd_conv_wgrad", C.byref(d), _stream(), nbytes=nbytes if _TIMING is not None else 0.0,
                tag=tag if TIMING_DETAIL else "")
    return part, S


def _wgrad_wino_entry(xs: Sequence[Tensor], dzs: Sequence[Tensor]):
    xb = min(x.data_ptr() for x in xs)
    zb = min(z.data_ptr() for z in dzs)
    xoff = tuple((x.data_ptr() - xb) // x.element_size() for x in xs)
    zoff = tuple((z.data_ptr() - zb) // z.element_size() for z in dzs)
    cache = _desc_cache()
    key = ("wgrad_wino", _geom(xs), _geom(dzs), xoff, zoff, COMPUTE, CU_RESERVE)
    ent = cache.get(key)
    if ent is None:
        d, _, flop, nbytes, tag, Cout, Cin, _ = _wgrad_desc(xs, dzs, 3, 1, 1, xoff, zoff)
        d.limbs3 = 1
        if COMPUTE != "f32x3" or not int(_lib.load().erd_conv_wgrad_wino_ok(C.byref(d))):
            ent = cache[key] = (None,)
        else:
            tiles = sum(dz.shape[0] * ((dz.shape[1] + 1) // 2) * ((dz.shape[2] + 1) // 2) for dz in dzs)
            comb = 4 * (Cout // 128) * (Cin // 128)
            steps = (tiles + 15) // 16
            S = int(max(1, min(_one_round(256) // comb, steps // 4 if steps >= 4 else 1)))
            nbytes += 4.0 * (S * 16 - d.nsplit * 9) * Cout * Cin
            d.nsplit = S
            ent = cache[key] = (d, S, flop, nbytes, tag.rsplit(" S", 1)[0] + f" S{S} wino", Cout, Cin)
    return ent, xb, zb


def conv_wgrad_wino_ok(xs: Sequence[Tensor], dzs: Sequence[Tensor]) -> bool:
    if COMPUTE != "f32x3" or any(t.dtype != torch.float32 for t in (*xs, *dzs)):
        return False
    return _wgrad_wino_entry(xs, dzs)[0][0] is not None


def conv_wgrad_wino(xs: Sequence[Tensor], dzs: Sequence[Tensor], nsplit: Optional[int] = None):
    _require_gpu(*xs, *dzs)
    ent, xb, zb = _wgrad_wino_entry(xs, dzs)
    if ent[0] is None:
        raise RuntimeError("conv_wgrad_wino: f32x3 mode, fp32 maps, 3x3 / stride 1 / pad 1, Cin and Cout multiples of 128 only")
    d, S, flop, nbytes, tag, Cout, Cin = ent
    if nsplit is not None:
        S = int(nsplit)
    d.nsplit = S
    d.x, d.dz = xb, zb
    part = ws_float("wgrad_part", S * 16 * Cout * Cin, xs[0].device)
    d.part = part.data_ptr()
    _timed_call("conv_wgrad_row3", flop, "erd_conv_wgrad_wino", C.byref(d), _stream(), nbytes=nbytes if _TIMING is not None else 0.0,
                tag=tag if TIMING_DETAIL else "")
    return part, S


def wgrad_wino_reduce(part: Tensor, S: int, dW: Tensor, accumulate: bool) -> None:
    Cout, Cin = dW.shape[0], dW.shape[-1]
    assert dW.numel() == Cout * 9 * Cin and dW.is_contiguous()
    call("erd_wgrad_wino_reduce", _p(part), S, Cout, Cin, _p(dW), 1 if accumulate else 0, _stream())


def _wgrad_desc(xs, dzs, k, stride, pad, xoff, zoff, ngroups: int = 1):
    Cin, Cout = xs[0].shape[3], dzs[0].shape[3]
    npix = sum(dz.shape[0] * dz.shape[1] * dz.shape[2] for dz in dzs)
    d = WgradDesc()
    xe = ze = 0
    d.nseg = len(xs)
    for i, (x, dz) in enumerate(zip(xs, dzs)):
        _check_map(x)
        _check_map(dz)
        sg = d.seg[i]
        _, nx = _extent(x)
        _, nz = _extent(dz)
        sg.x_off, sg.dz_off = xoff[i], zoff[i]
        xe, ze = max(xe, sg.x_off + nx), max(ze, sg.dz_off + nz)
        sg.N, sg.IH, sg.IW = x.shape[0], x.shape[1], x.shape[2]
        sg.GH, sg.GW, sg.OH, sg.OW = dz.shape[1], dz.shape[2], dz.shape[1], dz.shape[2]
        sg.x_nstride, sg.dz_nstride = x.stride(0), dz.stride(0)
    d.x_elems, d.dz_elems = xe, ze
    d.Cin, d.Cout, d.ntaps = Cin, Cout, k * k
    for kh in range(k):
        for kw in range(k):
            d.dy[kh * k + kw], d.dx[kh * k + kw] = kh - pad, kw - pad
    d.in_stride, d.out_stride, d.oy, d.ox = stride, 1, 0, 0
    d.bf16_multiplicands = 1 if COMPUTE == "bf16" else 0
    d.x_bf16, d.dz_bf16 = _stored_bf16(xs), _stored_bf16(dzs)
    row3 = int(_lib.load().erd_wgrad_row3_slices(C.byref(d))) if _os.environ.get("ERD_WGRAD_ROW3", "1") != "0" else 0
    d.limbs3 = 1 if (COMPUTE == "f32x3" and WGRAD_X3 and (row3 or WGRAD_X3_GENERIC)) else 0
    if row3 and d.limbs3:
        bmr = 128 if Cout > 64 else 64
        groups = ((Cout + bmr - 1) // bmr) * ((Cin + 63) // 64) * 3
        target = _one_round(int(_os.environ.get("ERD_WGRAD_ROW3_X3_TARGET", "768")))
        S = int(max(1, min(target // (groups * ngroups), row3 // 16 if row3 >= 16 else 1, 512)))
    elif row3:
        bme = 64 if Cout <= 64 else (96 if Cout <= 96 else 128)
        groups = ((Cout + bme - 1) // bme) * ((Cin + 127) // 128) * 3
        target = _one_round(int(_os.environ.get("ERD_WGRAD_ROW3_TARGET", "512")))
        S = int(max(1, min(target // groups, row3 // 16 if row3 >= 16 else 1, 512)))
    elif d.limbs3:
        tiles = ((Cout + 127) // 128) * ((Cin + 127) // 128) * k * k
        kt = (npix + 15) // 16
        S = int(max(1, min(_one_round(int(_os.environ.get("ERD_WGRAD_X3_TARGET", "768"))) // (tiles * ngroups), kt // 8 if kt >= 8 else 1, 512)))
    else:
        S = _pick_nsplit(npix, Cout, Cin, k * k)
    d.nsplit = S
    d.ngroups = ngroups
    flop = 2.0 * npix * Cout * Cin * k * k * ngroups
    nbytes = 4.0 * ngroups * (sum(t.numel() for t in xs) + sum(t.numel() for t in dzs) + S * Cout * k * k * Cin)
    tag = f"px{npix} {Cin}->{Cout} k{k}s{stride} S{S}" + (f" G{ngroups}" if ngroups > 1 else "")
    return d, S, flop, nbytes, tag, Cout, Cin, bool(row3)


def conv_wgrad_partials_grouped(xs_per_group: Sequence[Sequence[Tensor]], dzs_per_group: Sequence[Sequence[Tensor]], k: int, stride: int,
                                pad: int, nsplit: Optional[int] = None):
    G = len(xs_per_group)
    assert 1 <= G <= _lib.ERD_MAX_GROUPS and len(dzs_per_group) == G, f"1 .. {_lib.ERD_MAX_GROUPS} groups"
    xs0, dzs0 = xs_per_group[0], dzs_per_group[0]
    _require_gpu(*[t for xs in xs_per_group for t in xs], *[t for dzs in dzs_per_group for t in dzs])
    xbs = [min(x.data_ptr() for x in xs) for xs in xs_per_group]
    zbs = [min(z.data_ptr() for z in dzs) for dzs in dzs_per_group]
    offs = lambda ts, b: tuple((t.data_ptr() - b) // t.element_size() for t in ts)
    xoff, zoff = offs(xs0, xbs[0]), offs(dzs0, zbs[0])
    for g in range(1, G):
        assert (_geom(xs_per_group[g]), _geom(dzs_per_group[g]), offs(xs_per_group[g], xbs[g]), offs(dzs_per_group[g], zbs[g])) == \
            (_geom(xs0), _geom(dzs0), xoff, zoff), "the groups of a grouped weight gradient share one geometry"
    cache = _desc_cache()
    key = ("wgrad_grouped", G, k, stride, pad, _geom(xs0), _geom(dzs0), xoff, zoff, COMPUTE, _os.environ.get("ERD_WGRAD_ROW3", "1"), WGRAD_X3,
           WGRAD_X3_GENERIC, CU_RESERVE)
    ent = cache.get(key)
    if ent is None:
        ent = cache[key] = _wgrad_desc(xs0, dzs0, k, stride, pad, xoff, zoff, ngroups=G)
    d, S, flop, nbytes, tag, Cout, Cin, row3 = ent
    if not d.limbs3:
        raise RuntimeError("conv_wgrad_partials_grouped: only the three-limb weight-gradient kernels (compute mode f32x3) take groups")
    slab = Cout * k * k * Cin
    if nsplit is not None:
        nbytes += 4.0 * G * (int(nsplit) - S) * slab
        S = int(nsplit)
    d.nsplit = S
    d.x, d.dz = xbs[0], zbs[0]
    for g in range(G):
        d.gx[g], d.gdz[g] = xbs[g], zbs[g]
    part = ws_float("wgrad_part", G * S * slab, xs0[0].device)
    d.part = part.data_ptr()
    _timed_call("conv_wgrad_row3" if row3 else "conv_wgrad", flop, "erd_conv_wgrad", C.byref(d), _stream(), nbytes=nbytes if _TIMING is not None else 0.0,
                tag=tag if TIMING_DETAIL else "")
    return part, S


def wgrad_reduce_grouped(part: Tensor, S: int, ws: Sequence[Tensor], rowscales: Sequence[Optional[Tensor]], dWs: Sequence[Tensor],
                         accumulate: bool, rowdots: Sequence[Optional[Tensor]], rowdot_zeroed: bool = False) -> None:
    G = len(ws)
    assert 1 <= G <= _lib.ERD_MAX_GROUPS and len(rowscales) == len(dWs) == len(rowdots) == G
    Cout = ws[0].shape[0]
    Kd = ws[0].numel() // Cout
    t = _lib.WgradReduceGroups()
    t.ngroups = G
    for g in range(G):
        assert ws[g].shape == ws[0].shape and dWs[g].numel() == ws[0].numel()
        t.w[g] = ws[g].data_ptr()
        t.rowscale[g] = 0 if rowscales[g] is None else rowscales[g].data_ptr()
        t.dW[g] = dWs[g].data_ptr()
        t.rowdot[g] = 0 if rowdots[g] is None else rowdots[g].data_ptr()
    call("erd_wgrad_reduce_grouped", _p(part), S, Cout, Kd, C.byref(t), (1 if accumulate else 0) | (2 if rowdot_zeroed else 0), _stream())


def wgrad_reduce_rows(part: Tensor, S: int, Cout_slab: int, dW: Tensor, accumulate: bool) -> None:
    Cout = dW.shape[0]
    call("erd_wgrad_reduce_rows", _p(part), S, Cout_slab, Cout, dW.numel() // Cout, _p(dW), 1 if accumulate else 0,
         _stream())


def pad_channels(src: Tensor, Cp: int) -> Tensor:
    _require_gpu(src)
    assert src.dtype == torch.float32 and src.is_contiguous()
    C = src.shape[-1]
    out = torch.empty((*src.shape[:-1], Cp), dtype=torch.float32, device=src.device)
    call("erd_pad_channels", _p(src), _p(out), src.numel() // C, C, Cp, _stream())
    return out


def wgrad_reduce(part: Tensor, S: int, w: Tensor, rowscale: Optional[Tensor], dW: Tensor, accumulate: bool,
                 rowdot: Optional[Tensor], rowdot_zeroed: bool = False) -> None:
    Cout = w.shape[0]
    K = w.numel() // Cout
    call("erd_wgrad_reduce", _p(part), S, Cout, K, _p(w), _p(rowscale), _p(dW),
         (1 if accumulate else 0) | (2 if rowdot_zeroed else 0), _p(rowdot), _stream())


def stem(x_nchw: Tensor, w_ohwi: Tensor, scale: Tensor, shift: Tensor) -> Tensor:
    _require_gpu(x_nchw, w_ohwi)
    assert x_nchw.is_contiguous() and x_nchw.shape[1] == 3 and w_ohwi.shape == (64, 7, 7, 3) and w_ohwi.is_contiguous()
    N, _, H, W = x_nchw.shape
    OH, OW = conv_out_size(H, 7, 2, 3), conv_out_size(W, 7, 2, 3)
    y = torch.empty((N, OH, OW, 64), dtype=torch.float32, device=x_nchw.device)
    call("erd_stem_conv7x7_bn_relu", _p(x_nchw), _p(w_ohwi), _p(scale), _p(shift), _p(y), N, H, W, _stream())
    PH, PW = conv_out_size(OH, 3, 2, 1), conv_out_size(OW, 3, 2, 1)
    z = torch.empty((N, PH, PW, 64), dtype=act_dtype(), device=x_nchw.device)
    call("erd_maxpool3x3s2", _p(y), _p(z), N, OH, OW, 64, _mt(z), _stream())
    return z


def preprocess_into(img: Tensor, out_slot: Tensor, mean, std, flip_channels: bool, pad_value: float) -> None:
    _require_gpu(img, out_slot)
    assert img.dim() == 3 and img.shape[0] == 3 and img.is_contiguous() and out_slot.is_contiguous()
    assert img.dtype in (torch.uint8, torch.float32), img.dtype
    m = (C.c_float * 3)(*[float(v) for v in mean])
    s = (C.c_float * 3)(*[float(v) for v in std])
    call("erd_preprocess_image", _p(img), int(img.dtype == torch.uint8), img.shape[1], img.shape[2], _p(out_slot),
         out_slot.shape[1], out_slot.shape[2], m, s, int(flip_channels), float(pad_value), _stream())


def resize_normalize_into(src_hwc_u8: Tensor, tables, new_hw, out_slot: Tensor, mean, std, flip: bool, swap_rb: bool,
                          pad_value: float) -> None:
    _require_gpu(src_hwc_u8, out_slot)
    assert src_hwc_u8.dtype == torch.uint8 and src_hwc_u8.dim() == 3 and src_hwc_u8.shape[2] == 3 and src_hwc_u8.is_contiguous()
    xo, xc, yo, yc = tables
    m = (C.c_float * 3)(*[float(v) for v in mean])
    sd = (C.c_float * 3)(*[float(v) for v in std])
    call("erd_resize_normalize", _p(src_hwc_u8), src_hwc_u8.shape[0], src_hwc_u8.shape[1], _p(xo), _p(xc), _p(yo), _p(yc),
         int(new_hw[0]), int(new_hw[1]), _p(out_slot), out_slot.shape[1], out_slot.shape[2], m, sd, int(flip), int(swap_rb),
         float(pad_value), _stream())


RESIZE_ITEM_BYTES = C.sizeof(_lib.ResizeItem)


def resize_normalize_batch(packed_u8: Tensor, n: int, out: Tensor, mean, std, swap_rb: bool, pad_value: float,
                           table_offset: int = 0) -> None:
    _require_gpu(packed_u8, out)
    assert packed_u8.dtype == torch.uint8 and packed_u8.dim() == 1 and packed_u8.is_contiguous()
    assert out.dtype == torch.float32 and out.dim() == 4 and out.shape[0] == n and out.shape[1] == 3 and out.is_contiguous()
    assert table_offset % 8 == 0 and 0 <= table_offset and table_offset + n * RESIZE_ITEM_BYTES <= packed_u8.numel()
    m = (C.c_float * 3)(*[float(v) for v in mean])
    sd = (C.c_float * 3)(*[float(v) for v in std])
    call("erd_resize_normalize_batch", _p(packed_u8), packed_u8.numel(), packed_u8.data_ptr() + table_offset, n, _p(out),
         out.shape[2], out.shape[3], m, sd, int(swap_rb), float(pad_value), _stream())


def bn_fold(gamma: Tensor, beta: Tensor, mean: Tensor, var: Tensor, eps: float = 1e-5):
    _require_gpu(gamma)
    scale = torch.empty_like(gamma)
    shift = torch.empty_like(gamma)
    call("erd_bn_fold", _p(gamma), _p(beta), _p(mean), _p(var), eps, _p(scale), _p(shift), gamma.numel(), _stream())
    return scale, shift


def relu_bwd_colsum(y: Optional[Tensor], dy: Tensor, use_relu: bool, want_colsum: bool = True,
                    colsum_into: Optional[Tensor] = None):
    _check_map(dy)
    N, H, W, Cc = dy.shape
    colsum = colsum_into if colsum_into is not None else (zeros_f32(Cc, dy.device) if want_colsum else None)
    dz = dy
    if use_relu:
        _check_map(y)
        assert y.is_contiguous() and dy.is_contiguous(), "relu backward runs on dense maps"
        dz = torch.empty_like(dy)
    call("erd_relu_bwd_colsum", _p(y), _p(dy), _p(dz), N * H * W, Cc, dy.stride(0), H * W, _p(colsum),
         1 if use_relu else 0, _mt(dy, y if use_relu else None), _stream())
    return dz, colsum


COLSUM_COPIES = 8
COLSUM_WIDTH = int(_os.environ.get("ERD_COLSUM_WIDTH", "16384"))


def colsum_copies(channels: int) -> int:
    c = COLSUM_COPIES
    while COLSUM_WIDTH > 0 and c * 2 * channels <= COLSUM_WIDTH and c < 128:
        c *= 2
    return c


def bn_dgamma(rowdot: Tensor, dbeta: Tensor, mean: Tensor, var: Tensor, eps: float = 1e-5,
              out: Optional[Tensor] = None, dbeta_out: Optional[Tensor] = None) -> Tensor:
    Cc = dbeta.shape[-1]
    copies = dbeta.numel() // Cc
    dg = torch.empty(Cc, dtype=torch.float32, device=dbeta.device) if out is None else out
    call("erd_bn_dgamma", _p(rowdot), _p(dbeta), copies, _p(mean), _p(var), eps, _p(dg), _p(dbeta_out), 0, Cc, _stream())
    return dg


def colsum(x2d: Tensor, out: Optional[Tensor] = None) -> Tensor:
    assert x2d.is_contiguous()
    rows, Cc = x2d.shape[:-1].numel(), x2d.shape[-1]
    if out is None:
        out = torch.empty(Cc, dtype=torch.float32, device=x2d.device)
    call("erd_colsum", _p(x2d), rows, Cc, _p(out), 0, _mt(x2d), _stream())
    return out


def gn_relu_forward(c: Tensor, gamma: Tensor, beta: Tensor, sizes, G: int = 32, eps: float = 1e-5):
    _require_gpu(c)
    assert c.is_contiguous()
    N, A, Cc = c.shape
    lv = make_levels(sizes)
    y = torch.empty_like(c)
    nst = N * lv.nseg * G
    stats = workspace("gn_stats", nst * 16, c.device)
    mr = torch.empty((N, lv.nseg, G, 2), dtype=torch.float32, device=c.device)
    call("erd_gn_relu_fwd", _p(c), _p(y), _p(gamma), _p(beta), _p(stats), _p(mr), N, A, Cc, G, C.byref(lv), eps,
         _mt(c), _stream())
    return y, mr


GN_FUSED = _os.environ.get("ERD_GN_FUSED", "1") != "0"


def conv3x3_gn_relu_forward(x_cat: Tensor, w: Tensor, gamma: Tensor, beta: Tensor, sizes, G: int = 32, eps: float = 1e-5):
    _require_gpu(x_cat, w)
    N, A, Cin = x_cat.shape
    Cout = w.shape[0]
    c = torch.empty((N, A, Cout), dtype=x_cat.dtype, device=x_cat.device)
    xs, outs = level_views(x_cat, sizes), level_views(c, sizes)
    fused = (GN_FUSED and Cout == 256 and G == 32 and x_cat.dtype == torch.float32 and wino_ok(Cin, 3, 1, 1) and wino_x3()
             and (WINO_TRAIN_FWD if RECORDED else WINO_NOGRAD_FWD))
    ws_bytes = 0
    if fused:
        from ._lib import ConvSeg
        segs = (ConvSeg * len(xs))()
        for i, (x, o) in enumerate(zip(xs, outs)):
            _fill_seg(segs[i], x, o, x.shape[1], x.shape[2], None, None, None)
        ws_bytes = int(_lib.load().erd_wino_x3_gn_ws_bytes(segs, len(xs), Cout))
    if ws_bytes == 0:
        conv_forward(xs, w, outs, 3, 1, 1)
        y, mr = gn_relu_forward(c, gamma, beta, sizes, G, eps)
        return c, y, mr
    U = _wino_weights_cached(w)
    lv = make_levels(sizes)
    part = workspace("gn_part", ws_bytes, c.device)
    mr = torch.empty((N, lv.nseg, G, 2), dtype=torch.float32, device=c.device)
    flop = 2.0 * N * A * Cout * 9 * Cin
    nbytes = (4.0 * (x_cat.numel() + c.numel()) + U.numel() * U.element_size()) if _TIMING is not None else 0.0
    _timed_call("conv_wino_fwd_p", flop, "erd_wino_conv3x3_x3_gn", segs, len(xs), _p(U), Cin, Cout, None, None, 0,
                _p(_wino_sched(U.device)), _p(part), ws_bytes, _stream(), nbytes=nbytes,
                tag=f"px{N * A} {Cin}->{Cout} k3s1" if TIMING_DETAIL else "")
    call("erd_wino_gn_finalize", segs, len(xs), Cout, _p(part), _p(mr), eps, _stream())
    y = torch.empty_like(c)
    call("erd_gn_relu_apply", _p(c), _p(y), _p(gamma), _p(beta), _p(mr), N, A, Cout, G, C.byref(lv), _mt(c), _stream())
    return c, y, mr


def gn_relu_backward(c: Tensor, dy: Tensor, gamma: Tensor, beta: Tensor, mr: Tensor, sizes, G: int = 32,
                     dgamma: Optional[Tensor] = None, dbeta: Optional[Tensor] = None):
    assert c.is_contiguous() and dy.is_contiguous()
    N, A, Cc = c.shape
    lv = make_levels(sizes)
    stats = workspace("gn_stats", N * lv.nseg * G * 16, c.device)
    dc = torch.empty_like(c)
    dgamma = zeros_f32(gamma.numel(), c.device) if dgamma is None else dgamma
    dbeta = zeros_f32(beta.numel(), c.device) if dbeta is None else dbeta
    call("erd_gn_relu_bwd", _p(c), _p(dy), _p(gamma), _p(beta), _p(mr), _p(stats), _p(dc), _p(dgamma), _p(dbeta), N, A,
         Cc, G, C.byref(lv), _mt(c, dy), _stream())
    return dc, dgamma, dbeta


def upsample_add_(fine: Tensor, coarse: Tensor) -> None:
    _check_map(fine)
    _check_map(coarse)
    N, H, W, Cc = fine.shape
    call("erd_upsample2x_add", _p(fine), _p(coarse), N, H, W, Cc, coarse.shape[1], coarse.shape[2], fine.stride(0),
         coarse.stride(0), _mt(fine, coarse), _stream())
# ... 324 lines not shown
```

include/erd_hip.h:

```cpp
#ifndef ERD_HIP_H_
#define ERD_HIP_H_

#include <stddef.h>
#include <stdint.h>

#ifdef __cplusplus
extern "C" {
#endif

#define ERD_ABI_VERSION 6
#define ERD_MAX_SEG 5
#define ERD_MAX_TAPS 9
#define ERD_MAX_GROUPS 8

#define ERD_EINVAL (-1)
#define ERD_EUNSUPPORTED (-2)

typedef void* erd_stream_t;

enum { ERD_F32 = 0, ERD_BF16 = 1 };

int erd_abi_version(void);
int erd_set_cu_reserve(int n);
int erd_usable_cus(void);
int erd_probe_build(void);
const char* erd_last_error(void);
const char* erd_csrc_sha(void);

typedef struct {
    const float* in;
    float* out;
    const float* res;
    const float* alpha;
    const float* mask;
    int N, IH, IW, GH, GW, OH, OW;
    int64_t in_nstride, out_nstride, res_nstride;
    int tap0, ntaps, oy, ox;
} erd_conv_seg;

typedef struct {
    int nseg;
    erd_conv_seg seg[ERD_MAX_SEG];
    const float* w;
    int Cin, Cout, wrow;
    int ntaps;
    int dy[ERD_MAX_TAPS], dx[ERD_MAX_TAPS], wk[ERD_MAX_TAPS];
    int in_stride, out_stride, oy, ox;
    const float* scale;
    const float* shift;
    int relu;
    float* colsum;
    void* sk_ws;
    size_t sk_ws_bytes;
    const void* w_bf16;
    int colsum_copies;
    int in_bf16, out_bf16;
    const void* w_x3;
} erd_conv_desc;

int erd_conv_igemm(const erd_conv_desc* d, erd_stream_t stream);
size_t erd_conv_igemm_ws_bytes(int max_tiles);
int erd_conv_thin_enable(int on);
int erd_conv_thin_ok(const erd_conv_desc* d);
int erd_to_bf16(const float* src, void* dst, int64_t n, erd_stream_t stream);
int erd_split3(const float* src, void* dst, int64_t n, erd_stream_t stream);

size_t erd_wino_weights_elems(int Cout, int Cin);
int erd_wino_weights(const float* w_ohwi, float* U, int Cout, int Cin, int flip ,
                     erd_stream_t stream);
int erd_wino_conv3x3(const erd_conv_seg* segs, int nseg, const float* U, int Cin, int Cout, const float* scale,
                     const float* shift, int relu, float* colsum, int colsum_copies ,
                     int* sched ,
                     erd_stream_t stream);

size_t erd_wino_weights_x3_elems(int Cout, int Cin);
int erd_wino_weights_x3(const float* w_ohwi, void* U3, int Cout, int Cin, int flip, erd_stream_t stream);
int erd_wino_conv3x3_x3(const erd_conv_seg* segs, int nseg, const void* U3, int Cin, int Cout, const float* scale,
                        const float* shift, int relu, float* colsum, int colsum_copies, int* sched, erd_stream_t stream);
int erd_wino_x3_couts_per_item(const erd_conv_seg* segs, int nseg, int Cout);
int erd_wino_conv3x3_x3_gn(const erd_conv_seg* segs, int nseg, const void* U3, int Cin, int Cout, const float* scale,
                           const float* shift, int relu, int* sched, float* gn_part, size_t gn_part_bytes, erd_stream_t stream);
int erd_wino_gn_finalize(const erd_conv_seg* segs, int nseg, int Cout, const float* gn_part, float* mean_rstd, float eps,
                         erd_stream_t stream);
size_t erd_wino_x3_gn_ws_bytes(const erd_conv_seg* segs, int nseg, int Cout);

typedef struct {
    int64_t x_off, dz_off;
    int N, IH, IW, GH, GW, OH, OW;
    int64_t x_nstride, dz_nstride;
} erd_wgrad_seg;

typedef struct {
    const float* x;
    const float* dz;
    int64_t x_elems, dz_elems;
    int nseg;
    erd_wgrad_seg seg[ERD_MAX_SEG];
    int Cin, Cout, ntaps;
    int dy[ERD_MAX_TAPS], dx[ERD_MAX_TAPS];
    int in_stride, out_stride, oy, ox;
    float* part;
    int nsplit;
    int bf16_multiplicands;
    int x_bf16, dz_bf16;
    int limbs3;
    int ngroups;
    const float* gx[ERD_MAX_GROUPS];
    const float* gdz[ERD_MAX_GROUPS];
} erd_wgrad_desc;
int erd_conv_wgrad(const erd_wgrad_desc* d, erd_stream_t stream);
int erd_wgrad_row3_slices(const erd_wgrad_desc* d);

int erd_wgrad_reduce(const float* part, int nsplit, int Cout, int K, const float* w,
                     const float* rowscale, float* dW, int accumulate, float* rowdot,
                     erd_stream_t stream);
int erd_wgrad_reduce_rows(const float* part, int nsplit, int Cout_slab, int Cout, int K, float* dW, int accumulate,
                          erd_stream_t stream);
typedef struct {
    int ngroups;
    const float* w[ERD_MAX_GROUPS];
    const float* rowscale[ERD_MAX_GROUPS];
    float* dW[ERD_MAX_GROUPS];
    float* rowdot[ERD_MAX_GROUPS];
} erd_wgrad_reduce_groups;
int erd_wgrad_reduce_grouped(const float* part, int nsplit, int Cout, int K, const erd_wgrad_reduce_groups* groups,
                             int accumulate, erd_stream_t stream);

int erd_conv_wgrad_wino(const erd_wgrad_desc* d, erd_stream_t stream);
int erd_conv_wgrad_wino_ok(const erd_wgrad_desc* d);
int erd_conv_wgrad_wino_tile(const erd_wgrad_desc* d);
int erd_wgrad_wino_reduce(const float* part, int nsplit, int Cout, int Cin, float* dW, int accumulate, erd_stream_t stream);

typedef struct {
    const float* in;
    float* out;
    const float* w;
    const float* scale;
    const float* shift;
    const float* res;
    const float* mask;
    float* colsum;
    int colsum_copies;
    int N, IH, IW, OH, OW;
    int C, cg, stride, relu;
} erd_conv_grouped_desc;
int erd_conv_grouped_fwd(const erd_conv_grouped_desc* d, erd_stream_t stream);
int erd_conv_grouped_dgrad(const erd_conv_grouped_desc* d, erd_stream_t stream);
int erd_conv_grouped_wgrad(const float* x, const float* dz, float* part, int N, int IH, int IW, int C, int cg, int stride,
                           int nsplit, erd_stream_t stream);
int erd_conv_grouped_wgrad_splits(int N, int IH, int IW, int C, int cg, int stride);

int erd_deform_cols(const float* x, const float* offset, float* col, int N, int IH, int IW, int C, int stride, erd_stream_t stream);
int erd_deform_cols_bwd(const float* dcol, const float* x, const float* offset, float* dx, float* doffset, int N, int IH, int IW,
                        int C, int stride, erd_stream_t stream);

int erd_weight_transpose(const float* w, const float* rowscale, float* dst, int Cout, int ntaps,
                         int Cin, int flip, erd_stream_t stream);
int erd_weight_transpose_bf16(const float* w, const float* rowscale, void* dst, int Cout, int ntaps,
                              int Cin, int flip, erd_stream_t stream);
int erd_weight_transpose_x3(const float* w, const float* rowscale, void* dst, int Cout, int ntaps,
                            int Cin, int flip, erd_stream_t stream);

typedef struct {
    const float* w;
    const float* rowscale;
    void* dst;
    int Cout, ntaps, Cin, flip;
    int kind;
    int block0;
} erd_weight_prep_item;
int erd_weight_prep_blocks(int kind, int Cout, int ntaps, int Cin);
int erd_weight_prep_batch(const erd_weight_prep_item* items_dev, int nitems, int total_blocks, erd_stream_t stream);

int erd_stem_conv7x7_bn_relu(const float* x_nchw, const float* w_ohwi, const float* scale,
                             const float* shift, float* out_nhwc, int N, int H, int W,
                             erd_stream_t stream);
int erd_maxpool3x3s2(const float* in, void* out, int N, int H, int W, int C, int out_type ,
                     erd_stream_t stream);

int erd_preprocess_image(const void* img, int is_uint8, int h, int w, float* out, int H, int W,
                         const float* mean3, const float* std3, int flip_channels, float pad_value,
                         erd_stream_t stream);

int erd_resize_normalize(const void* src_hwc_u8, int sh, int sw, const int* xofs, const short* xcoef,
                         const int* yofs, const short* ycoef, int nh, int nw, float* out, int H, int W,
                         const float* mean3, const float* std3, int flip, int swap_rb, float pad_value,
                         erd_stream_t stream);
typedef struct {
    int64_t offset;
    int sh, sw;
    int nh, nw;
    int flip;
    int reserved;
} erd_resize_item;
int erd_resize_normalize_batch(const void* src_u8, int64_t src_bytes, const erd_resize_item* items_dev, int n, float* out,
                               int H, int W, const float* mean3, const float* std3, int swap_rb, float pad_value,
                               erd_stream_t stream);

int erd_bn_fold(const float* gamma, const float* beta, const float* mean, const float* var,
                float eps, float* scale, float* shift, int64_t n, erd_stream_t stream);
typedef struct {
    const float* gamma;
    const float* beta;
    const float* mean;
    const float* var;
    float* scale;
    float* shift;
    int n;
    float eps;
} erd_bn_fold_item;
int erd_bn_fold_batch(const erd_bn_fold_item* items_dev, int nitems, int max_n, erd_stream_t stream);
int erd_relu_bwd_colsum(const void* y, const void* dy, void* dz, int64_t npix, int C,
                        int64_t nstride_rows, int64_t rows_per_img, float* colsum, int use_relu,
                        int map_type , erd_stream_t stream);
int erd_bn_dgamma(const float* rowdot, const float* dbeta, int copies, const float* mean, const float* var,
                  float eps, float* dgamma, float* dbeta_out, int accumulate, int C, erd_stream_t stream);

typedef struct {
    int nseg;
    int64_t off[ERD_MAX_SEG];
    int64_t cnt[ERD_MAX_SEG];
} erd_levels;
int erd_gn_relu_fwd(const void* c, void* y, const float* gamma, const float* beta, double* stats_ws,
                    float* mean_rstd, int N, int64_t A, int C, int G, const erd_levels* lv, float eps,
                    int map_type , erd_stream_t stream);
int erd_gn_relu_apply(const void* c, void* y, const float* gamma, const float* beta, const float* mean_rstd, int N,
                      int64_t A, int C, int G, const erd_levels* lv, int map_type , erd_stream_t stream);
int erd_gn_relu_bwd(const void* c, const void* dy, const float* gamma, const float* beta,
                    const float* mean_rstd, double* stats_ws, void* dc, float* dgamma, float* dbeta,
                    int N, int64_t A, int C, int G, const erd_levels* lv, int map_type ,
                    erd_stream_t stream);

int erd_upsample2x_add(void* fine, const void* coarse, int N, int H, int W, int C, int h, int w,
                       int64_t fine_nstride, int64_t coarse_nstride, int map_type, erd_stream_t stream);
int erd_upsample2x_add_bwd(const void* dfine, void* dcoarse, int N, int H, int W, int C, int h, int w,
                           int64_t fine_nstride, int64_t coarse_nstride, int map_type, erd_stream_t stream);

int erd_colsum(const void* x, int64_t rows, int C, float* out, int accumulate, int map_type , erd_stream_t stream);
int erd_pad_channels(const float* src, float* dst, int64_t rows, int C, int Cp, erd_stream_t stream);
int erd_level_scale(const float* x, const float* alphas, float* y, int N, int64_t A, int C,
                    const erd_levels* lv, erd_stream_t stream);
int erd_level_scale_bwd(const float* x, const float* dy, const float* alphas, float* dx, float* dalphas,
                        int N, int64_t A, int C, const erd_levels* lv, erd_stream_t stream);
int erd_sgd_momentum(float* p, const float* g, float* buf, int64_t n, float lr, float momentum,
                     float weight_decay, float grad_scale, int first_step, erd_stream_t stream);

typedef struct {
    int64_t begin;
    float lr_mult;
    float weight_decay;
} erd_sgd_seg;
int erd_sgd_groups_table(const int64_t* seg_off, const float* lr_mult, const float* weight_decay, int nseg,
                         erd_sgd_seg* table_dev, erd_stream_t stream);
int erd_sgd_momentum_groups(float* p, const float* g, float* buf, int64_t base, int64_t n, const erd_sgd_seg* table_dev,
                            int seg0, int nseg, int64_t seg0_begin, int64_t seg_end, float lr, float momentum,
                            float grad_scale, const float* clip_coef, int first_step, erd_stream_t stream);
int erd_adam_groups(float* p, const float* g, float* exp_avg, float* exp_avg_sq, int64_t base, int64_t n,
                    const erd_sgd_seg* table_dev, int seg0, int nseg, int64_t seg0_begin, int64_t seg_end, float lr,
                    float weight_decay, double beta1, double beta2, float eps, float inv_bias1, float inv_sqrt_bias2,
                    float grad_scale, const float* clip_coef, int decoupled, erd_stream_t stream);
#define ERD_SQNORM_PARTS 1024
int erd_grad_sqnorm(const float* g, int64_t n, double* partials, erd_stream_t stream);
int erd_clip_coef(const double* partials, int nslots, float grad_scale, float max_norm, float* out, erd_stream_t stream);
int erd_grad_accumulate(float* acc, const float* g, int64_t n, int first, erd_stream_t stream);

int erd_ers_select(const float* cls, const float* bbox, int N, int64_t A, int Ccls, int Cbox,
                   uint8_t* mask_cls, uint8_t* mask_bbox, int64_t* idx_cls, int64_t* idx_bbox,
                   int32_t* counts, float* thr, double* ws, erd_stream_t stream);

int erd_grid_anchors(float* anchors, const int* hs, const int* ws, const int* strides, int nlvl,
                     int octave_scale, erd_stream_t stream);
int erd_atss_assign(const float* anchors, const uint8_t* valid, const int64_t* lvl_off, int nlvl,
                    int64_t A, const float* gt_boxes, const int64_t* gt_labels, const int32_t* gt_off,
                    int N, int max_gt, int topk, int num_classes, int64_t* labels, float* label_weights,
                    float* bbox_targets, int32_t* num_pos, void* ws, erd_stream_t stream);

int erd_gfl_losses_fwd(const float* cls, const float* bbox, const float* anchors, const int64_t* labels,
                       const float* label_weights, const float* bbox_targets, const int64_t* lvl_off,
                       const int* strides, int nlvl, int N, int64_t A, int c_old, int c_all,
                       float* score_ws, float* wt_ws, double* out_sums, erd_stream_t stream);
int erd_gfl_losses_bwd(const float* cls, const float* bbox, const float* anchors, const int64_t* labels,
                       const float* label_weights, const float* bbox_targets, const int64_t* lvl_off,
                       const int* strides, int nlvl, int N, int64_t A, int c_old, int c_all,
                       const float* score_ws, const float* wt_ws, const float* coef ,
                       float* dcls, float* dbbox, erd_stream_t stream);

int erd_l2_distill(const float* s_cls, const float* t_cls, const int64_t* idx_cls, const int32_t* counts,
                   int N, int64_t A, int c_s, int c_t, int c_old, double* sums, erd_stream_t stream);
int erd_l2_distill_bwd(const float* s_cls, const float* t_cls, const int64_t* idx_cls,
                       const int32_t* counts, const float* coef, int N, int64_t A, int c_s, int c_t,
                       int c_old, float* dcls, erd_stream_t stream);
int erd_distill_nms(const float* t_cls, const float* t_bbox, const float* anchors,
                    const int64_t* idx_bbox, const int32_t* counts, int N, int64_t A, int c_t,
                    float iou_thr, uint8_t* keep_mask, int32_t* keep_count, float* ws, size_t ws_bytes,
                    erd_stream_t stream);
int erd_kd_kl(const float* s_bbox, const float* t_bbox, const float* s_cls, const uint8_t* keep_mask,
              int N, int64_t A, int c_s, int c_old, float T, double* sums, erd_stream_t stream);
int erd_kd_kl_bwd(const float* s_bbox, const float* t_bbox, const float* s_cls, const uint8_t* keep_mask,
                  const float* coef, int N, int64_t A, int c_s, int c_old, float T, float* dbbox,
                  erd_stream_t stream);

int erd_loss_finalize(const double* lvl_sums, const float* avg, const double* l2_sums, const double* kd_sums,
                      const int32_t* counts, int nlvl, int N, int c_old, float dist_loss_weight,
                      float lw_cls, float lw_bbox, float lw_dfl, float lw_ld, const float* upstream,
                      float* losses, float* coef, erd_stream_t stream);

int erd_loss_avg(const int32_t* num_pos, int N, const double* lvl_sums, int nlvl, float* avg,
                 erd_stream_t stream);

size_t erd_predict_ws_bytes(int N, int nlvl, int nms_pre);
int erd_predict_topk(const float* cls, const float* bbox, const float* anchors, int N, int64_t A, int C,
                     const erd_levels* lv, const int* strides, const float* img_hw, float score_thr,
                     int nms_pre, float* boxes, float* scores, int32_t* labels, int32_t* num, void* ws,
                     size_t ws_bytes, erd_stream_t stream);
int erd_predict_nms(const float* boxes, const float* scores, const int32_t* labels, const int32_t* num,
                    int N, int max_cols, const float* inv_scale, float min_bbox_size, float iou_thr,
                    int max_per_img, float* dets, int64_t* det_labels, int32_t* det_num, void* ws,
                    size_t ws_bytes, erd_stream_t stream);
size_t erd_tta_merge_ws_bytes(int V, int N, int P);
int erd_tta_merge(const float* dets, const int64_t* labels, const int32_t* num, int V, int N, int P,
                  const int32_t* flip, const float* ori_w, float iou_thr, int max_per_img, float* out_dets,
                  int64_t* out_labels, int32_t* out_num, void* ws, size_t ws_bytes, erd_stream_t stream);

int erd_coco_dets_append(const float* dets, const int64_t* labels, const int32_t* num, const int32_t* img_index, int N, int P,
                         double* box, double* score, int32_t* img, int32_t* label, erd_stream_t stream);
size_t erd_coco_eval_ws_bytes(int64_t D, int npairs, int K, int64_t ngt);
int erd_coco_eval(const double* dt_box, const double* dt_score, const int32_t* dt_img, const int32_t* dt_label, int64_t D,
                  const double* gt_box, const double* gt_area, const int32_t* gt_flag, const int32_t* gt_off, int I, int K,
                  int64_t ngt, const int32_t* n_gt, const double* area_rng, const double* iou_start, const double* rec_thrs,
                  const int32_t* max_dets, double* precision, double* recall, void* ws, size_t ws_bytes, erd_stream_t stream);

int erd_qfl_rows(const float* pred, const int64_t* label, const float* score, int64_t n, int C, float* rows, erd_stream_t stream);
int erd_qfl_bwd(const float* pred, const int64_t* label, const float* score, const float* coef, int64_t n, int C, float* dpred,
                erd_stream_t stream);
int erd_dfl(const float* pred, const float* target, const float* coef, int64_t m, int nb, float* rows, float* dpred,
            erd_stream_t stream);
int erd_kd_kl_rows(const float* pred, const float* soft, const float* coef, int64_t m, int nb, float T, float* rows, float* dpred,
                   erd_stream_t stream);
int erd_giou(const float* pred, const float* target, const float* coef, int64_t n, float eps, float* rows, float* dpred,
             erd_stream_t stream);
int erd_bbox_overlaps(const float* b1, const float* b2, int64_t A, int64_t G, int aligned, int mode, float eps, float* out,
                      erd_stream_t stream);
int erd_integral(const float* x, const float* dy, int64_t m, int nb, float* y, float* dx, erd_stream_t stream);
int erd_distance2bbox(const float* points, const float* dist, const float* dout, int64_t n, float max_h, float max_w, float* out,
                      float* ddist, erd_stream_t stream);
int erd_bbox2distance(const float* points, const float* boxes, int64_t n, float max_dis, float eps, float* out, erd_stream_t stream);
int erd_weighted_sum(const float* rows, const float* weight, int64_t n, double scale, float* out, erd_stream_t stream);
int erd_loss_coef(const float* upstream, const float* weight, int64_t n, float scale, float* coef, erd_stream_t stream);
int erd_rows_mul(const float* rows, const float* weight, int64_t n, float scale, float* out, erd_stream_t stream);
int erd_atss_result(const void* assign_ws, const int64_t* gt_labels, int64_t A, int64_t* gt_inds, float* max_overlaps,
                    int64_t* labels, erd_stream_t stream);

#ifdef __cplusplus
}
#endif
#endif
```

Measured before the change: 126.7 images/sec.

## Extend Winograd weight-gradient path to grouped, non-128 Cout, and BN-fused reduce

Generalizes the Winograd-domain weight-gradient kernels so they accept several weight groups in one launch, output-channel counts that are multiples of 4 (padded to 128-row slabs with masked loads), and a reduce epilogue that applies a per-row scale and accumulates the weight·grad row dot product. Head and conv_module weight gradients are routed through this path when a heuristic (Cin>=256 and enough tiles) says it pays. The aim is to replace slower direct wgrad and separate BN-fold/rowdot passes with the cheaper Winograd form, plus fewer launches. The cost is padded partial buffers, extra masked work for small Cout, and an atomic per row in the reduce.

```diff
diff --git a/erd_amd/_lib.py b/erd_amd/_lib.py
--- a/erd_amd/_lib.py
+++ b/erd_amd/_lib.py
@@ -117,6 +117,8 @@
     "erd_conv_wgrad_wino_ok": [C.POINTER(WgradDesc)],
     "erd_conv_wgrad_wino_tile": [C.POINTER(WgradDesc)],
     "erd_wgrad_wino_reduce": [P, i32, i32, i32, P, i32, P],
+    "erd_wgrad_wino_reduce_bn": [P, i32, i32, i32, i32, P, P, P, i32, P, P],
+    "erd_wgrad_wino_reduce_grouped": [P, i32, i32, i32, i32, C.POINTER(WgradReduceGroups), i32, P],
     "erd_weight_transpose": [P, P, P, i32, i32, i32, i32, P],
     "erd_weight_transpose_bf16": [P, P, P, i32, i32, i32, i32, P],
     "erd_stem_conv7x7_bn_relu": [P, P, P, P, P, i32, i32, i32, P],
diff --git a/erd_amd/csrc/wgrad_wino.hip b/erd_amd/csrc/wgrad_wino.hip
--- a/erd_amd/csrc/wgrad_wino.hip
+++ b/erd_amd/csrc/wgrad_wino.hip
@@ -143,6 +143,19 @@
     }
 };
 
+__device__ __forceinline__ void group_of(const erd_wgrad_desc& p, int slab, int& split, const float*& bx, const float*& bz) {
+    split = slab;
+    bx = p.x;
+    bz = p.dz;
+    if (p.ngroups > 1) {
+        const int grp = slab / p.nsplit;
+        split = slab - grp * p.nsplit;
+#pragma unroll
+        for (int g = 0; g < ERD_MAX_GROUPS; ++g)
+            if (g == grp) { bx = p.gx[g]; bz = p.gdz[g]; }
+    }
+}
+
 __global__ __launch_bounds__(WT) void conv_wgrad_wino_kernel(const erd_wgrad_desc p, const int ntiles, const int nsteps) {
     extern __shared__ __attribute__((aligned(16))) char smem[];
     unsigned* tab = reinterpret_cast<unsigned*>(smem + OPER_BYTES);
@@ -150,9 +163,12 @@
     const int tid = threadIdx.x, wave = tid >> 6, lane = tid & 63;
     const int wave_u = __builtin_amdgcn_readfirstlane(wave);
 
-    const int nci = p.Cin / BC, nco = p.Cout / BC, ncomb = 4 * nci * nco;
+    const int nci = p.Cin / BC, nco = (p.Cout + BC - 1) / BC, ncomb = 4 * nci * nco;
     const int wg = erd::xcd_contiguous(blockIdx.x, gridDim.x);
-    const int split = wg / ncomb, comb = wg - split * ncomb;
+    const int slab = wg / ncomb, comb = wg - slab * ncomb;
+    int split;
+    const float *base_x, *base_z;
+    group_of(p, slab, split, base_x, base_z);
     const int r = comb & 3, ct = comb >> 2;
     const int ci0 = (ct % nci) * BC, co0 = (ct / nci) * BC;
     const int per = (nsteps + p.nsplit - 1) / p.nsplit;
@@ -164,9 +180,9 @@
     TileTable tt{p, rs, rs, tab, lane, ntiles};
 
     const int cg = (wave & 3) * 16 + (lane & 15), tp = (wave >> 2) * 4 + (lane >> 4);
-    const __amdgpu_buffer_rsrc_t rs_x = __builtin_amdgcn_make_buffer_rsrc(const_cast<float*>(p.x), 0, (int)(p.x_elems * 4), 0x00020000);
-    const __amdgpu_buffer_rsrc_t rs_z = __builtin_amdgcn_make_buffer_rsrc(const_cast<float*>(p.dz), 0, (int)(p.dz_elems * 4), 0x00020000);
-    const unsigned chan_x = (unsigned)(ci0 + 2 * cg) * 4u, chan_z = (unsigned)(co0 + 2 * cg) * 4u;
+    const __amdgpu_buffer_rsrc_t rs_x = __builtin_amdgcn_make_buffer_rsrc(const_cast<float*>(base_x), 0, (int)(p.x_elems * 4), 0x00020000);
+    const __amdgpu_buffer_rsrc_t rs_z = __builtin_amdgcn_make_buffer_rsrc(const_cast<float*>(base_z), 0, (int)(p.dz_elems * 4), 0x00020000);
+    const unsigned chan_x = (unsigned)(ci0 + 2 * cg) * 4u, chan_z = co0 + 2 * cg < p.Cout ? (unsigned)(co0 + 2 * cg) * 4u : INV;
     const unsigned step_x = (unsigned)p.Cin * 4u, step_z = (unsigned)p.Cout * 4u;
     float2 rx[16], rz[8];
 #pragma unroll
@@ -293,7 +309,7 @@
         }
     }
 
-    float* __restrict__ part = p.part + ((int64_t)(split * 16 + 4 * r + pj) * p.Cout) * p.Cin;
+    float* __restrict__ part = p.part + ((int64_t)(slab * 16 + 4 * r + pj) * (nco * BC)) * p.Cin;
 #pragma unroll
     for (int i = 0; i < 2; ++i)
 #pragma unroll
@@ -322,9 +338,12 @@
     const int tid = threadIdx.x, wave = tid >> 6, lane = tid & 63;
     const int wave_u = __builtin_amdgcn_readfirstlane(wave);
 
-    const int nci = p.Cin / BP, nco = p.Cout / BP, ncomb = 16 * nci * nco;
+    const int nci = p.Cin / BP, nco = (p.Cout + BP - 1) / BP, ncomb = 16 * nci * nco;
     const int wg = erd::xcd_contiguous(blockIdx.x, gridDim.x);
-    const int split = wg / ncomb, comb = wg - split * ncomb;
+    const int slab = wg / ncomb, comb = wg - slab * ncomb;
+    int split;
+    const float *base_x, *base_z;
+    group_of(p, slab, split, base_x, base_z);
     const int xi = comb & 15, ct = comb >> 4;
     const int ci0 = (ct % nci) * BP, co0 = (ct / nci) * BP;
     const int per = (nsteps + p.nsplit - 1) / p.nsplit;
@@ -337,9 +356,10 @@
     TileTable tt{p, rs, cs, tab, lane, ntiles};
 
     const int cg = wave * 16 + (lane & 15), tq = lane >> 4;
-    const __amdgpu_buffer_rsrc_t rs_x = __builtin_amdgcn_make_buffer_rsrc(const_cast<float*>(p.x), 0, (int)(p.x_elems * 4), 0x00020000);
-    const __amdgpu_buffer_rsrc_t rs_z = __builtin_amdgcn_make_buffer_rsrc(const_cast<float*>(p.dz), 0, (int)(p.dz_elems * 4), 0x00020000);
+    const __amdgpu_buffer_rsrc_t rs_x = __builtin_amdgcn_make_buffer_rsrc(const_cast<float*>(base_x), 0, (int)(p.x_elems * 4), 0x00020000);
+    const __amdgpu_buffer_rsrc_t rs_z = __builtin_amdgcn_make_buffer_rsrc(const_cast<float*>(base_z), 0, (int)(p.dz_elems * 4), 0x00020000);
     const unsigned chan = (unsigned)cg * 8u, tile_x = (unsigned)ci0 * 4u, tile_z = (unsigned)co0 * 4u;
+    const unsigned chan_z = co0 + 2 * cg < p.Cout ? chan : INV;
     float2 rx[16], rz[16];
 #pragma unroll
     for (int i = 0; i < 16; ++i) rz[i] = make_float2(0.f, 0.f);
@@ -356,17 +376,17 @@
 #pragma unroll
             for (int i = 0; i < 4; ++i) rx[q * 4 + i] = buf_load8(rs_x, ox[q][i] + chan, tile_x);
 #pragma unroll
-        for (int q = 0; q < 4; ++q) rz[q * 4] = buf_load8(rs_z, oz[q][0] + chan, tile_z);
+        for (int q = 0; q < 4; ++q) rz[q * 4] = buf_load8(rs_z, __builtin_elementwise_add_sat(oz[q][0], chan_z), tile_z);
         if (zc_two) {
 #pragma unroll
-            for (int q = 0; q < 4; ++q) rz[q * 4 + 1] = buf_load8(rs_z, oz[q][1] + chan, tile_z);
+            for (int q = 0; q < 4; ++q) rz[q * 4 + 1] = buf_load8(rs_z, __builtin_elementwise_add_sat(oz[q][1], chan_z), tile_z);
         }
         if (z_two) {
 #pragma unroll
-            for (int q = 0; q < 4; ++q) rz[q * 4 + 2] = buf_load8(rs_z, oz[q][2] + chan, tile_z);
+            for (int q = 0; q < 4; ++q) rz[q * 4 + 2] = buf_load8(rs_z, __builtin_elementwise_add_sat(oz[q][2], chan_z), tile_z);
             if (zc_two) {
 #pragma unroll
-                for (int q = 0; q < 4; ++q) rz[q * 4 + 3] = buf_load8(rs_z, oz[q][3] + chan, tile_z);
+                for (int q = 0; q < 4; ++q) rz[q * 4 + 3] = buf_load8(rs_z, __builtin_elementwise_add_sat(oz[q][3], chan_z), tile_z);
             }
         }
     };
@@ -461,7 +481,7 @@
         }
     }
 
-    float* __restrict__ part = p.part + ((int64_t)(split * 16 + xi) * p.Cout) * p.Cin;
+    float* __restrict__ part = p.part + ((int64_t)(slab * 16 + xi) * (nco * BP)) * p.Cin;
 #pragma unroll
     for (int i = 0; i < 2; ++i)
 #pragma unroll
@@ -473,15 +493,25 @@
         }
 }
 
-__global__ __launch_bounds__(256) void wgrad_wino_reduce_kernel(const float* __restrict__ part, int nsplit, int Cout, int Cin,
-                                                                 float* __restrict__ dW, int accumulate) {
+__global__ __launch_bounds__(256) void wgrad_wino_reduce_kernel(const float* __restrict__ part, int nsplit, int Cout_slab, int Cin,
+                                                                 const float* __restrict__ w, const float* __restrict__ rowscale,
+                                                                 float* __restrict__ dW, int accumulate, float* __restrict__ rowdot,
+                                                                 const erd_wgrad_reduce_groups groups) {
     __shared__ float4 du[16][16];
+    __shared__ float red[4];
     const int co = blockIdx.x, xi = threadIdx.x >> 4, c4 = threadIdx.x & 15;
     const int ci = blockIdx.y * 64 + c4 * 4;
-    const int64_t slab = (int64_t)16 * Cout * Cin;
+    const int64_t slab = (int64_t)16 * Cout_slab * Cin;
+    if (groups.ngroups > 0) {
+        const int g = blockIdx.z;
+        part += (int64_t)g * nsplit * slab;
+#pragma unroll
+        for (int i = 0; i < ERD_MAX_GROUPS; ++i)
+            if (i == g) { w = groups.w[i]; rowscale = groups.rowscale[i]; dW = groups.dW[i]; rowdot = groups.rowdot[i]; }
+    }
     float4 s = make_float4(0.f, 0.f, 0.f, 0.f);
     if (ci < Cin) {
-        const float* src = part + ((int64_t)xi * Cout + co) * Cin + ci;
+        const float* src = part + ((int64_t)xi * Cout_slab + co) * Cin + ci;
         for (int k = 0; k < nsplit; ++k) {
             const float4 v = *reinterpret_cast<const float4*>(src + k * slab);
             s.x += v.x; s.y += v.y; s.z += v.z; s.w += v.w;
@@ -489,27 +519,44 @@
     }
     du[xi][c4] = s;
     __syncthreads();
-    if (threadIdx.x >= 9 * 16 || ci >= Cin) return;
-    const int a = xi / 3, b = xi - 3 * a;
-    auto col = [&](int i) {
-        const float4 u1 = du[4 * i + 1][c4], u2 = du[4 * i + 2][c4];
-        if (b == 1) return make_float4(u1.x - u2.x, u1.y - u2.y, u1.z - u2.z, u1.w - u2.w);
-        const float4 u0 = du[4 * i + (b == 0 ? 0 : 3)][c4];
-        return make_float4((u1.x + u2.x) + u0.x, (u1.y + u2.y) + u0.y, (u1.z + u2.z) + u0.z, (u1.w + u2.w) + u0.w);
-    };
-    const float4 e1 = col(1), e2 = col(2);
-    float4 o;
-    if (a == 1) o = make_float4(e1.x - e2.x, e1.y - e2.y, e1.z - e2.z, e1.w - e2.w);
-    else {
-        const float4 e0 = col(a == 0 ? 0 : 3);
-        o = make_float4((e1.x + e2.x) + e0.x, (e1.y + e2.y) + e0.y, (e1.z + e2.z) + e0.z, (e1.w + e2.w) + e0.w);
-    }
-    float* dst = dW + ((int64_t)co * 9 + xi) * Cin + ci;
-    if (accumulate) {
-        const float4 old = *reinterpret_cast<const float4*>(dst);
-        o.x += old.x; o.y += old.y; o.z += old.z; o.w += old.w;
-    }
-    *reinterpret_cast<float4*>(dst) = o;
+    float dot = 0.f;
+    if (threadIdx.x < 9 * 16 && ci < Cin) {
+        const int a = xi / 3, b = xi - 3 * a;
+        auto col = [&](int i) {
+            const float4 u1 = du[4 * i + 1][c4], u2 = du[4 * i + 2][c4];
+            if (b == 1) return make_float4(u1.x - u2.x, u1.y - u2.y, u1.z - u2.z, u1.w - u2.w);
+            const float4 u0 = du[4 * i + (b == 0 ? 0 : 3)][c4];
+            return make_float4((u1.x + u2.x) + u0.x, (u1.y + u2.y) + u0.y, (u1.z + u2.z) + u0.z, (u1.w + u2.w) + u0.w);
+        };
+        const float4 e1 = col(1), e2 = col(2);
+        float4 o;
+        if (a == 1) o = make_float4(e1.x - e2.x, e1.y - e2.y, e1.z - e2.z, e1.w - e2.w);
+        else {
+            const float4 e0 = col(a == 0 ? 0 : 3);
+            o = make_float4((e1.x + e2.x) + e0.x, (e1.y + e2.y) + e0.y, (e1.z + e2.z) + e0.z, (e1.w + e2.w) + e0.w);
+        }
+        const int64_t at = ((int64_t)co * 9 + xi) * Cin + ci;
+        if (rowdot) {
+            const float4 ww = *reinterpret_cast<const float4*>(w + at);
+            dot = ww.x * o.x + ww.y * o.y + ww.z * o.z + ww.w * o.w;
+        }
+        if (rowscale) {
+            const float rs = rowscale[co];
+            o = make_float4(rs * o.x, rs * o.y, rs * o.z, rs * o.w);
+        }
+        float* dst = dW + at;
+        if (accumulate) {
+            const float4 old = *reinterpret_cast<const float4*>(dst);
+            o.x += old.x; o.y += old.y; o.z += old.z; o.w += old.w;
+        }
+        *reinterpret_cast<float4*>(dst) = o;
+    }
+    if (rowdot) {
+        dot = erd::wave_sum(dot);
+        if ((threadIdx.x & 63) == 0) red[threadIdx.x >> 6] = dot;
+        __syncthreads();
+        if (threadIdx.x == 0) atomicAdd(rowdot + co, (red[0] + red[1]) + red[2]);
+    }
 }
 
 int64_t wino_tiles(const erd_wgrad_desc* d) {
@@ -518,8 +565,9 @@
     return n;
 }
 
+int cout_slab(const erd_wgrad_desc* d) { return (d->Cout + BC - 1) / BC * BC; }
 int wino_tile(const erd_wgrad_desc* d) {
-    const bool can = d->Cin % BP == 0 && d->Cout % BP == 0;
+    const bool can = d->Cin % BP == 0 && cout_slab(d) % BP == 0;
     const char* const e = getenv("ERD_WGRAD_WINO_TILE");
     const int force = e ? atoi(e) : 0;
     if (force == BC || !can) return BC;
@@ -531,23 +579,33 @@
 extern "C" int erd_conv_wgrad_wino_tile(const erd_wgrad_desc* d) { return erd_conv_wgrad_wino_ok(d) ? wino_tile(d) : 0; }
 
 extern "C" int erd_conv_wgrad_wino_ok(const erd_wgrad_desc* d) {
-    if (!d || d->bf16_multiplicands || d->x_bf16 || d->dz_bf16 || d->ngroups != 1) return 0;
-    if (d->nseg < 1 || d->nseg > ERD_MAX_SEG || d->Cin < BC || d->Cout < BC || d->Cin % BC || d->Cout % BC) return 0;
+    if (!d || d->bf16_multiplicands || d->x_bf16 || d->dz_bf16 || d->ngroups < 1 || d->ngroups > ERD_MAX_GROUPS) return 0;
+    if (d->nseg < 1 || d->nseg > ERD_MAX_SEG || d->Cin < BC || d->Cout < 4 || d->Cin % BC || d->Cout % 4) return 0;
     if (d->x_elems <= 0 || d->dz_elems <= 0 || d->x_elems >= (1ll << 29) || d->dz_elems >= (1ll << 29)) return 0;
-    for (int l = 0; l < d->nseg; ++l)
-        if (d->seg[l].N < 1 || d->seg[l].GH < 1 || d->seg[l].GW < 1) return 0;
+    for (int l = 0; l < d->nseg; ++l) {
+        const erd_wgrad_seg& g = d->seg[l];
+        if (g.N < 1 || g.GH < 1 || g.GW < 1) return 0;
+        if (g.dz_off < 0 || g.dz_off + (g.N - 1) * g.dz_nstride + (int64_t)g.OH * g.OW * d->Cout > d->dz_elems) return 0;
+    }
+    if (d->ngroups > 1)
+        for (int g = 0; g < d->ngroups; ++g)
+            if (!d->gx[g] || !d->gdz[g]) return 0;
     return erd_wgrad_row3_slices(d) > 0 && wino_tiles(d) < (1ll << 30);
 }
 
 extern "C" int erd_conv_wgrad_wino(const erd_wgrad_desc* d, erd_stream_t stream) {
-    ERD_REQUIRE(d != nullptr && d->part && d->x && d->dz, "wgrad_wino: null pointer");
+    ERD_REQUIRE(d != nullptr && d->part, "wgrad_wino: null pointer");
+    ERD_REQUIRE(d->ngroups >= 1 && d->ngroups <= ERD_MAX_GROUPS, "wgrad_wino: ngroups=%d", d->ngroups);
+    if (d->ngroups == 1) ERD_REQUIRE(d->x && d->dz, "wgrad_wino: null pointer");
+    else
+        for (int g = 0; g < d->ngroups; ++g) ERD_REQUIRE(d->gx[g] && d->gdz[g], "wgrad_wino: null pointer in group %d", g);
     ERD_REQUIRE(!d->bf16_multiplicands && !d->x_bf16 && !d->dz_bf16, "wgrad_wino: fp32 maps and the three-limb form only");
-    ERD_REQUIRE(d->ngroups == 1, "wgrad_wino: ngroups=%d", d->ngroups);
-    ERD_REQUIRE(d->Cin >= BC && d->Cout >= BC && d->Cin % BC == 0 && d->Cout % BC == 0, "wgrad_wino: Cin=%d Cout=%d must be multiples of %d", d->Cin,
-                d->Cout, BC);
+    ERD_REQUIRE(d->Cin >= BC && d->Cin % BC == 0, "wgrad_wino: Cin=%d must be a multiple of %d", d->Cin, BC);
+    ERD_REQUIRE(d->Cout >= 4 && d->Cout % 4 == 0, "wgrad_wino: Cout=%d must be a multiple of 4", d->Cout);
     ERD_REQUIRE(d->in_stride == 1 && d->out_stride == 1, "wgrad_wino: stride 1 only");
-    ERD_REQUIRE(erd_conv_wgrad_wino_ok(d), "wgrad_wino: not a 3x3 / stride 1 / pad 1 layer over 1 .. %d non-empty maps below 2 GiB", ERD_MAX_SEG);
-    const int64_t grid = (int64_t)4 * (d->Cin / BC) * (d->Cout / BC) * d->nsplit;
+    ERD_REQUIRE(erd_conv_wgrad_wino_ok(d), "wgrad_wino: not a 3x3 / stride 1 / pad 1 layer over 1 .. %d non-empty maps inside their extents below 2 GiB",
+                ERD_MAX_SEG);
+    const int64_t grid = (int64_t)4 * (d->Cin / BC) * (cout_slab(d) / BC) * d->nsplit * d->ngroups;
     ERD_REQUIRE(d->nsplit >= 1 && grid < (1 << 20), "wgrad_wino: nsplit=%d", d->nsplit);
     const int ntiles = (int)wino_tiles(d), nsteps = (ntiles + KT - 1) / KT;
     static bool attr_done = false;
@@ -563,7 +621,33 @@
 
 extern "C" int erd_wgrad_wino_reduce(const float* part, int nsplit, int Cout, int Cin, float* dW, int accumulate, erd_stream_t stream) {
     ERD_REQUIRE(part && dW && nsplit >= 1 && Cout >= 1 && Cin >= 4 && Cin % 4 == 0, "wgrad_wino_reduce: bad args");
-    hipLaunchKernelGGL(wgrad_wino_reduce_kernel, dim3(Cout, (Cin + 63) / 64), dim3(256), 0, (hipStream_t)stream, part, nsplit, Cout, Cin, dW,
-                       accumulate & 1);
+    hipLaunchKernelGGL(wgrad_wino_reduce_kernel, dim3(Cout, (Cin + 63) / 64), dim3(256), 0, (hipStream_t)stream, part, nsplit, Cout, Cin, nullptr,
+                       nullptr, dW, accumulate & 1, nullptr, erd_wgrad_reduce_groups{});
     return erd::check_launch("wgrad_wino_reduce");
 }
+
+extern "C" int erd_wgrad_wino_reduce_bn(const float* part, int nsplit, int Cout_slab, int Cout, int Cin, const float* w, const float* rowscale,
+                                        float* dW, int accumulate, float* rowdot, erd_stream_t stream) {
+    ERD_REQUIRE(part && dW && nsplit >= 1 && Cout >= 1 && Cout <= Cout_slab && Cin >= 4 && Cin % 4 == 0, "wgrad_wino_reduce_bn: bad args");
+    ERD_REQUIRE(!rowdot || w, "wgrad_wino_reduce_bn: rowdot needs w");
+    if (rowdot && !(accumulate & 2)) (void)hipMemsetAsync(rowdot, 0, sizeof(float) * Cout, (hipStream_t)stream);
+    hipLaunchKernelGGL(wgrad_wino_reduce_kernel, dim3(Cout, (Cin + 63) / 64), dim3(256), 0, (hipStream_t)stream, part, nsplit, Cout_slab, Cin, w,
+                       rowscale, dW, accumulate & 1, rowdot, erd_wgrad_reduce_groups{});
+    return erd::check_launch("wgrad_wino_reduce_bn");
+}
+
+extern "C" int erd_wgrad_wino_reduce_grouped(const float* part, int nsplit, int Cout_slab, int Cout, int Cin, const erd_wgrad_reduce_groups* groups,
+                                             int accumulate, erd_stream_t stream) {
+    ERD_REQUIRE(part && groups && nsplit >= 1 && Cout >= 1 && Cout <= Cout_slab && Cin >= 4 && Cin % 4 == 0, "wgrad_wino_reduce_grouped: bad args");
+    ERD_REQUIRE(groups->ngroups >= 1 && groups->ngroups <= ERD_MAX_GROUPS, "wgrad_wino_reduce_grouped: ngroups=%d", groups->ngroups);
+    for (int g = 0; g < groups->ngroups; ++g) {
+        ERD_REQUIRE(groups->dW[g], "wgrad_wino_reduce_grouped: group %d has no dW", g);
+        ERD_REQUIRE(!groups->rowdot[g] || groups->w[g], "wgrad_wino_reduce_grouped: rowdot of group %d needs w", g);
+    }
+    if (!(accumulate & 2))
+        for (int g = 0; g < groups->ngroups; ++g)
+            if (groups->rowdot[g]) (void)hipMemsetAsync(groups->rowdot[g], 0, sizeof(float) * Cout, (hipStream_t)stream);
+    hipLaunchKernelGGL(wgrad_wino_reduce_kernel, dim3(Cout, (Cin + 63) / 64, groups->ngroups), dim3(256), 0, (hipStream_t)stream, part, nsplit,
+                       Cout_slab, Cin, nullptr, nullptr, nullptr, accumulate & 1, nullptr, *groups);
+    return erd::check_launch("wgrad_wino_reduce_grouped");
+}
diff --git a/erd_amd/functional.py b/erd_amd/functional.py
--- a/erd_amd/functional.py
+++ b/erd_amd/functional.py
@@ -146,15 +146,27 @@
     return _to_oihw(dWk)
 
 
-def _emit_wgrad_wino(w: Tensor, part: Tensor, S: int, wk: Tensor):
+def _emit_wgrad_wino(w: Tensor, part: Tensor, S: int, wk: Tensor, scale: Optional[Tensor] = None, rowdot: Optional[Tensor] = None):
     sink = _sink(w)
     if sink is not None:
-        K.wgrad_wino_reduce(part, S, ohwi(sink), True)
+        K.wgrad_wino_reduce(part, S, ohwi(sink), True, wk, scale, rowdot, rowdot_zeroed=True)
         _sunk(w)
         return None
     dWk = torch.empty_like(wk)
-    K.wgrad_wino_reduce(part, S, dWk, False)
+    K.wgrad_wino_reduce(part, S, dWk, False, wk, scale, rowdot, rowdot_zeroed=True)
     return _to_oihw(dWk)
+
+
+def _wino_route(xin: Tensor, dz: Tensor, k: int, s: int, pad: int, card: int = 1, ngroups: int = 1) -> bool:
+    return WGRAD_WINO and card == 1 and (k, s, pad) == (3, 1, 1) and K.conv_wgrad_wino_ok([xin], [dz], ngroups, coupled=True)
+
+
+def _wgrad_coupled(w: Tensor, xin: Tensor, dz: Tensor, k: int, s: int, pad: int, card: int, wk: Tensor, scale: Tensor, rowdot: Optional[Tensor]):
+    if _wino_route(xin, dz, k, s, pad, card):
+        part, S = K.conv_wgrad_wino([xin], [dz])
+        return _emit_wgrad_wino(w, part, S, wk, scale, rowdot)
+    part, S = K.conv_wgrad_partials([xin], [dz], k, s, pad, cardinality=card)
+    return _emit_wgrad(w, part, S, wk, scale, rowdot)
 
 
 class _WgradGroups:
@@ -188,10 +200,15 @@
             return
         _, _, _, k, s, pad = q[0][:6]
         with (_Trail(self.dev, *[t for m in q for t in (m[1], m[2], m[6], m[7])]) if WGRAD_TRAIL else _contextlib.nullcontext()):
-            part, S = K.conv_wgrad_partials_grouped([[m[1]] for m in q], [[m[2]] for m in q], k, s, pad)
+            wino = _wino_route(q[0][1], q[0][2], k, s, pad, 1, len(q))
+            if wino:
+                part, S = K.conv_wgrad_wino_grouped([[m[1]] for m in q], [[m[2]] for m in q])
+            else:
+                part, S = K.conv_wgrad_partials_grouped([[m[1]] for m in q], [[m[2]] for m in q], k, s, pad)
             wks = [ohwi(m[8][0]) for m in q]
             rowdots = [K.zeros_f32(m[6].numel(), m[6].device) if m[9][1] else None for m in q]
-            K.wgrad_reduce_grouped(part, S, wks, [m[6] for m in q], [ohwi(_sink(m[8][0])) for m in q], True, rowdots, rowdot_zeroed=True)
+            (K.wgrad_wino_reduce_grouped if wino else K.wgrad_reduce_grouped)(part, S, wks, [m[6] for m in q], [ohwi(_sink(m[8][0])) for m in q],
+                                                                                True, rowdots, rowdot_zeroed=True)
             for m, rowdot in zip(q, rowdots):
                 (w, g, b, mean, var), (_, need_g, need_b), dbeta = m[8], m[9], m[7]
                 _sunk(w)
@@ -351,8 +368,7 @@
             rowdot = K.zeros_f32(scale.numel(), scale.device) if need_g else None
             dgamma = torch.empty_like(scale) if need_g else None
             with fork:
-                part, S = K.conv_wgrad_partials([x], [dz], k, stride, pad, cardinality=card)
-                dW = _emit_wgrad(w, part, S, wk, scale, rowdot)
+                dW = _wgrad_coupled(w, x, dz, k, stride, pad, card, wk, scale, rowdot)
                 if need_g:
                     K.bn_dgamma(rowdot, dbeta, mean, var, eps, out=dgamma)
         dx = None
@@ -508,9 +524,8 @@
                 trail.__exit__(None, None, None)
 
     def _wgrad_body(idx, xin, dz, k, s, pad, scale, dbeta, w, g, b, m, v, base, wk, card=1):
-        part, S = K.conv_wgrad_partials([xin], [dz], k, s, pad, cardinality=card)
         rowdot = K.zeros_f32(scale.numel(), scale.device) if need_p[base + 1] else None
-        grads[5 * idx] = _emit_wgrad(w, part, S, wk, scale, rowdot)
+        grads[5 * idx] = _wgrad_coupled(w, xin, dz, k, s, pad, card, wk, scale, rowdot)
         if need_p[base + 1]:
             rep = dbeta.dim() == 2
             bs_fold = (_sink(b) if need_p[base + 2] else None) if rep else None
diff --git a/erd_amd/kernels.py b/erd_amd/kernels.py
--- a/erd_amd/kernels.py
+++ b/erd_amd/kernels.py
@@ -1010,57 +1010,112 @@
     return part, S
 
 
-def _wgrad_wino_entry(xs: Sequence[Tensor], dzs: Sequence[Tensor]):
+def _wino_slab_rows(Cout: int) -> int:
+    return (Cout + 127) // 128 * 128
+
+
+WGRAD_WINO_MIN_TILES = 1024
+
+
+def wgrad_wino_pays(Cin: int, Cout: int, tiles: int, ngroups: int = 1, coupled: bool = False) -> bool:
+    if ngroups == 1 and Cout % 128 == 0 and not coupled:
+        return True
+    return Cin >= 256 and tiles >= WGRAD_WINO_MIN_TILES
+
+
+def _wgrad_wino_entry(xs: Sequence[Tensor], dzs: Sequence[Tensor], ngroups: int = 1):
     xb = min(x.data_ptr() for x in xs)
     zb = min(z.data_ptr() for z in dzs)
     xoff = tuple((x.data_ptr() - xb) // x.element_size() for x in xs)
     zoff = tuple((z.data_ptr() - zb) // z.element_size() for z in dzs)
     cache = _desc_cache()
-    key = ("wgrad_wino", _geom(xs), _geom(dzs), xoff, zoff, COMPUTE, CU_RESERVE)
+    key = ("wgrad_wino", ngroups, _geom(xs), _geom(dzs), xoff, zoff, COMPUTE, CU_RESERVE)
     ent = cache.get(key)
     if ent is None:
-        d, _, flop, nbytes, tag, Cout, Cin, _ = _wgrad_desc(xs, dzs, 3, 1, 1, xoff, zoff)
+        d, _, flop, nbytes, tag, Cout, Cin, _ = _wgrad_desc(xs, dzs, 3, 1, 1, xoff, zoff, ngroups=ngroups)
         d.limbs3 = 1
+        for g in range(ngroups if ngroups > 1 else 0):
+            d.gx[g], d.gdz[g] = xb, zb
         if COMPUTE != "f32x3" or not int(_lib.load().erd_conv_wgrad_wino_ok(C.byref(d))):
             ent = cache[key] = (None,)
         else:
             tiles = sum(dz.shape[0] * ((dz.shape[1] + 1) // 2) * ((dz.shape[2] + 1) // 2) for dz in dzs)
-            comb = 4 * (Cout // 128) * (Cin // 128)
+            rows = _wino_slab_rows(Cout)
+            comb = 4 * (rows // 128) * (Cin // 128) * ngroups
             steps = (tiles + 15) // 16
             S = int(max(1, min(_one_round(256) // comb, steps // 4 if steps >= 4 else 1)))
-            nbytes += 4.0 * (S * 16 - d.nsplit * 9) * Cout * Cin
+            nbytes += 4.0 * ngroups * (S * 16 * rows - d.nsplit * 9 * Cout) * Cin
             d.nsplit = S
-            ent = cache[key] = (d, S, flop, nbytes, tag.rsplit(" S", 1)[0] + f" S{S} wino", Cout, Cin)
+            ent = cache[key] = (d, S, flop, nbytes, tag.rsplit(" S", 1)[0] + f" S{S}" + (f" G{ngroups}" if ngroups > 1 else "") + " wino", Cout, Cin, tiles)
     return ent, xb, zb
 
 
-def conv_wgrad_wino_ok(xs: Sequence[Tensor], dzs: Sequence[Tensor]) -> bool:
+def conv_wgrad_wino_ok(xs: Sequence[Tensor], dzs: Sequence[Tensor], ngroups: int = 1, coupled: bool = False) -> bool:
     if COMPUTE != "f32x3" or any(t.dtype != torch.float32 for t in (*xs, *dzs)):
         return False
-    return _wgrad_wino_entry(xs, dzs)[0][0] is not None
+    ent = _wgrad_wino_entry(xs, dzs, ngroups)[0]
+    return ent[0] is not None and wgrad_wino_pays(ent[6], ent[5], ent[7], ngroups, coupled)
 
 
 def conv_wgrad_wino(xs: Sequence[Tensor], dzs: Sequence[Tensor], nsplit: Optional[int] = None):
-    _require_gpu(*xs, *dzs)
-    ent, xb, zb = _wgrad_wino_entry(xs, dzs)
+    return conv_wgrad_wino_grouped([xs], [dzs], nsplit)
+
+
+def conv_wgrad_wino_grouped(xs_per_group: Sequence[Sequence[Tensor]], dzs_per_group: Sequence[Sequence[Tensor]], nsplit: Optional[int] = None):
+    G = len(xs_per_group)
+    assert 1 <= G <= _lib.ERD_MAX_GROUPS and len(dzs_per_group) == G, f"1 .. {_lib.ERD_MAX_GROUPS} groups"
+    xs, dzs = xs_per_group[0], dzs_per_group[0]
+    _require_gpu(*[t for q in xs_per_group for t in q], *[t for q in dzs_per_group for t in q])
+    ent, xb, zb = _wgrad_wino_entry(xs, dzs, G)
     if ent[0] is None:
-        raise RuntimeError("conv_wgrad_wino: f32x3 mode, fp32 maps, 3x3 / stride 1 / pad 1, Cin and Cout multiples of 128 only")
-    d, S, flop, nbytes, tag, Cout, Cin = ent
+        raise RuntimeError("conv_wgrad_wino: f32x3 mode, fp32 maps, 3x3 / stride 1 / pad 1, Cin a multiple of 128 and Cout of 4 only")
+    d, S, flop, nbytes, tag, Cout, Cin, _ = ent
     if nsplit is not None:
         S = int(nsplit)
     d.nsplit = S
     d.x, d.dz = xb, zb
-    part = ws_float("wgrad_part", S * 16 * Cout * Cin, xs[0].device)
+    if G > 1:
+        offs = lambda ts, b: tuple((t.data_ptr() - b) // t.element_size() for t in ts)
+        for g in range(G):
+            gxb, gzb = min(x.data_ptr() for x in xs_per_group[g]), min(z.data_ptr() for z in dzs_per_group[g])
+            assert (_geom(xs_per_group[g]), _geom(dzs_per_group[g]), offs(xs_per_group[g], gxb), offs(dzs_per_group[g], gzb)) == \
+                (_geom(xs), _geom(dzs), offs(xs, xb), offs(dzs, zb)), "the groups of a grouped weight gradient share one geometry"
+            d.gx[g], d.gdz[g] = gxb, gzb
+    part = ws_float("wgrad_part", G * S * 16 * _wino_slab_rows(Cout) * Cin, xs[0].device)
     d.part = part.data_ptr()
     _timed_call("conv_wgrad_row3", flop, "erd_conv_wgrad_wino", C.byref(d), _stream(), nbytes=nbytes if _TIMING is not None else 0.0,
                 tag=tag if TIMING_DETAIL else "")
     return part, S
 
 
-def wgrad_wino_reduce(part: Tensor, S: int, dW: Tensor, accumulate: bool) -> None:
+def wgrad_wino_reduce(part: Tensor, S: int, dW: Tensor, accumulate: bool, w: Optional[Tensor] = None, rowscale: Optional[Tensor] = None,
+                      rowdot: Optional[Tensor] = None, rowdot_zeroed: bool = False) -> None:
     Cout, Cin = dW.shape[0], dW.shape[-1]
     assert dW.numel() == Cout * 9 * Cin and dW.is_contiguous()
-    call("erd_wgrad_wino_reduce", _p(part), S, Cout, Cin, _p(dW), 1 if accumulate else 0, _stream())
+    if rowscale is None and rowdot is None and _wino_slab_rows(Cout) == Cout:
+        call("erd_wgrad_wino_reduce", _p(part), S, Cout, Cin, _p(dW), 1 if accumulate else 0, _stream())
+        return
+    assert rowdot is None or w is not None
+    call("erd_wgrad_wino_reduce_bn", _p(part), S, _wino_slab_rows(Cout), Cout, Cin, _p(w), _p(rowscale), _p(dW),
+         (1 if accumulate else 0) | (2 if rowdot_zeroed else 0), _p(rowdot), _stream())
+
+
+def wgrad_wino_reduce_grouped(part: Tensor, S: int, ws: Sequence[Tensor], rowscales: Sequence[Optional[Tensor]], dWs: Sequence[Tensor],
+                              accumulate: bool, rowdots: Sequence[Optional[Tensor]], rowdot_zeroed: bool = False) -> None:
+    G = len(ws)
+    assert 1 <= G <= _lib.ERD_MAX_GROUPS and len(rowscales) == len(dWs) == len(rowdots) == G
+    Cout, Cin = ws[0].shape[0], ws[0].shape[-1]
+    assert ws[0].numel() == Cout * 9 * Cin
+    t = _lib.WgradReduceGroups()
+    t.ngroups = G
+    for g in range(G):
+        assert ws[g].shape == ws[0].shape and dWs[g].numel() == ws[0].numel()
+        t.w[g] = ws[g].data_ptr()
+        t.rowscale[g] = 0 if rowscales[g] is None else rowscales[g].data_ptr()
+        t.dW[g] = dWs[g].data_ptr()
+        t.rowdot[g] = 0 if rowdots[g] is None else rowdots[g].data_ptr()
+    call("erd_wgrad_wino_reduce_grouped", _p(part), S, _wino_slab_rows(Cout), Cout, Cin, C.byref(t),
+         (1 if accumulate else 0) | (2 if rowdot_zeroed else 0), _stream())
 
 
 def _wgrad_desc(xs, dzs, k, stride, pad, xoff, zoff, ngroups: int = 1):
diff --git a/include/erd_hip.h b/include/erd_hip.h
--- a/include/erd_hip.h
+++ b/include/erd_hip.h
@@ -130,6 +130,10 @@
 int erd_conv_wgrad_wino_ok(const erd_wgrad_desc* d);
 int erd_conv_wgrad_wino_tile(const erd_wgrad_desc* d);
 int erd_wgrad_wino_reduce(const float* part, int nsplit, int Cout, int Cin, float* dW, int accumulate, erd_stream_t stream);
+int erd_wgrad_wino_reduce_bn(const float* part, int nsplit, int Cout_slab, int Cout, int Cin, const float* w, const float* rowscale,
+                             float* dW, int accumulate, float* rowdot, erd_stream_t stream);
+int erd_wgrad_wino_reduce_grouped(const float* part, int nsplit, int Cout_slab, int Cout, int Cin,
+                                  const erd_wgrad_reduce_groups* groups, int accumulate, erd_stream_t stream);
 
 typedef struct {
     const float* in;
```

Result: no change. 127.1 images/sec, median of 6 (+0.3%).
